# hugocornellier/face_detection_tflite

Measured on NVIDIA B200. Metric: images/sec BlazeFace detect (pre+infer+NMS), higher is better.
Workload: dtype f32

## Files before the change

face_detection_tflite_b200/csrc/engine.cu:

```cuda
#include "engine.h"

#include <algorithm>
#include <cstdio>
#include <cstdlib>

namespace fdt {

Engine::~Engine() {
  if (d_blob_) cudaFree(d_blob_);
  for (TailLayerD* p : d_tail_) if (p) cudaFree(p);
  for (TailBlk* p : d_blks_) if (p) cudaFree(p);
}

bool Engine::init(const uint8_t* tflite, size_t len, int fuse_level, std::string* err, bool use_tc) {
  if (!model_.parse(tflite, len, err)) return false;
  if (!plan_.build(model_, fuse_level, err, use_tc)) return false;
  size_t bytes = plan_.blob.size() * sizeof(float) + 64;
  if (cudaMalloc(&d_blob_, bytes) != cudaSuccess) { *err = "cudaMalloc(weights) failed"; return false; }
  cudaMemset(d_blob_, 0, bytes);
  if (cudaMemcpy(d_blob_, plan_.blob.data(), plan_.blob.size() * sizeof(float), cudaMemcpyHostToDevice) != cudaSuccess) {
    *err = "weight upload failed";
    return false;
  }
  d_tail_.assign(plan_.steps.size(), nullptr);
  d_blks_.assign(plan_.steps.size(), nullptr);
  for (size_t i = 0; i < plan_.steps.size(); ++i) {
    const PStep& st = plan_.steps[i];
    if (st.kind != kStepTailWs) continue;
    if (cudaMalloc(&d_tail_[i], st.tail.size() * sizeof(TailLayerD)) != cudaSuccess ||
        cudaMemcpy(d_tail_[i], st.tail.data(), st.tail.size() * sizeof(TailLayerD), cudaMemcpyHostToDevice) != cudaSuccess) {
      *err = "tail program upload failed";
      return false;
    }
    if (st.tail_blks.empty()) continue;
    if (cudaMalloc(&d_blks_[i], st.tail_blks.size() * sizeof(TailBlk)) != cudaSuccess ||
        cudaMemcpy(d_blks_[i], st.tail_blks.data(), st.tail_blks.size() * sizeof(TailBlk), cudaMemcpyHostToDevice) != cudaSuccess) {
      *err = "chain block table upload failed";
      return false;
    }
  }
  return true;
}

bool Engine::make_ctx(int cap, EngineCtx* ctx, std::string* err) const {
  ctx->cap = cap;
  size_t bytes = (size_t)cap * plan_.arena_per_image * sizeof(float) + 256;
  if (cudaMalloc(&ctx->arena, bytes) != cudaSuccess) { *err = "cudaMalloc(arena) failed"; return false; }
  cudaMemset(ctx->arena, 0, bytes);
  ctx->outputs.clear();
  for (long long e : plan_.out_elems) {
    float* p = nullptr;
    size_t ob = (size_t)cap * e * sizeof(float) + 256;
    if (cudaMalloc(&p, ob) != cudaSuccess) { *err = "cudaMalloc(outputs) failed"; return false; }
    cudaMemset(p, 0, ob);
    ctx->outputs.push_back(p);
  }
  return true;
}

void Engine::free_ctx(EngineCtx* ctx) const {
  if (ctx->arena) cudaFree(ctx->arena);
  for (float* p : ctx->outputs) cudaFree(p);
  ctx->arena = nullptr;
  ctx->outputs.clear();
}

TV Engine::view(const EngineCtx& ctx, int t) const {
  const PTensor& x = plan_.tensors[t];
  TV v;
  v.H = x.H; v.W = x.W; v.C = x.C; v.Cs = x.Cs;
  v.istride = x.istride;
  if (x.root >= 0) v.p = ctx.outputs[x.root] + x.view_off;
  else v.p = ctx.arena + (size_t)x.arena_off * ctx.cap;
  return v;
}

static int cta_cap(size_t smem, int threads) {
  int by_smem = (int)((227u * 1024u) / (smem + 1024u));
  int by_thr = 2048 / std::max(threads, 32);
  int per_sm = std::max(1, std::min(std::min(by_smem, by_thr), 16));
  return 148 * per_sm;
}

int Engine::run(const EngineCtx& ctx, const uint8_t* in_u8, int B, cudaStream_t s, cudaEvent_t* evs) const {
  int launches = 0;
  const float* blob = d_blob_;
  for (const PStep& st : plan_.steps) {
    if (evs) cudaEventRecord(evs[launches], s);
    TV out = view(ctx, st.out);
    switch (st.kind) {
      case kStepNormalize:
        launch_normalize(in_u8, out, B, s);
        break;
      case kStepNaiveConv: {
        NaiveConvP p;
        p.in = view(ctx, st.in); p.out = out;
        p.w = blob + st.w; p.bias = blob + st.bias;
        p.alpha = st.alpha >= 0 ? blob + st.alpha : nullptr;
        p.kh = st.kh; p.kw = st.kw; p.sh = st.sh; p.sw = st.sw; p.pt = st.pt; p.pl = st.pl;
        p.act = st.act; p.depthwise = st.depthwise;
        launch_naive_conv(p, B, s);
        break;
      }
      case kStepStem: {
        StemP p;
        const PTensor& it = plan_.tensors[st.in];
        p.in8 = in_u8; p.H = it.H; p.W = it.W; p.OH = out.H; p.OW = out.W;
        p.kw = st.kw; p.pt = st.pt; p.pl = st.pl; p.K = st.K; p.KP = st.KP;
        p.out = out.p; p.out_istride = out.istride; p.Cout = st.Cout; p.CoutS = out.Cs;
        p.vec_store = (out.Cs % 4 == 0 && out.istride % 4 == 0 && ((size_t)out.p % 16 == 0)) ? ((out.Cs % 8 == 0 && out.istride % 8 == 0 && ((size_t)out.p % 32 == 0)) ? 2 : 1) : 0;
        p.w = blob + st.w; p.bias = blob + st.bias; p.alpha = st.alpha >= 0 ? blob + st.alpha : nullptr;
        p.act = st.act; p.CoutP = st.CoutP; p.NC = st.NC; p.smem_bytes = st.smem;
        launch_stem(p, B, s, cta_cap(st.smem, 32 * (st.NC / 4)));
        break;
      }
      case kStepStemWs: {
        StemWsP p;
        const PTensor& it = plan_.tensors[st.in];
        p.in8 = in_u8; p.H = it.H; p.W = it.W; p.OH = out.H; p.OW = out.W;
        p.kw = st.kw; p.pt = st.pt; p.pl = st.pl;
        p.out = out.p; p.out_istride = out.istride; p.Cout = st.Cout; p.CoutS = out.Cs;
        p.vec_store = (out.Cs % 4 == 0 && out.istride % 4 == 0 && ((size_t)out.p % 16 == 0)) ? ((out.Cs % 8 == 0 && out.istride % 8 == 0 && ((size_t)out.p % 32 == 0)) ? 2 : 1) : 0;
        p.wB = blob + st.w; p.bias = blob + st.bias; p.alpha = st.alpha >= 0 ? blob + st.alpha : nullptr;
        p.act = st.act; p.Npad = st.Npad; p.K8 = st.K8; p.tmem_cols = st.tmem_cols; p.w_parts = st.w_parts;
        p.out_scale = (float)st.out_scale; p.smem_bytes = st.smem;
        if (!launch_stem_ws(p, B, ctx.cap, s)) { failed_ = true; fprintf(stderr, "fdt: cuTensorMapEncodeTiled failed for step '%s'\n", st.name.c_str()); }
        break;
      }
      case kStepGemmConv: {
        GemmConvP p;
        const PTensor& it = plan_.tensors[st.in];
        if (st.in_u8) {
          p.in = nullptr; p.in8 = in_u8; p.in_istride = (long long)it.H * it.W * 4;
          p.Cin = 3; p.CinS = 3;
        } else {
          TV iv = view(ctx, st.in);
          p.in = iv.p; p.in8 = nullptr; p.in_istride = iv.istride; p.Cin = it.C; p.CinS = it.Cs;
        }
        p.H = it.H; p.W = it.W;
        p.kh = st.kh; p.kw = st.kw; p.sh = st.sh; p.sw = st.sw; p.pt = st.pt; p.pl = st.pl;
        p.OH = out.H; p.OW = out.W;
        p.K = st.K; p.KP = st.KP; p.KS = st.KS;
        p.out = out.p; p.out_istride = out.istride; p.Cout = st.Cout; p.CoutS = out.Cs;
        p.vec_store = (out.Cs % 4 == 0 && out.istride % 4 == 0 && ((size_t)out.p % 16 == 0)) ? ((out.Cs % 8 == 0 && out.istride % 8 == 0 && ((size_t)out.p % 32 == 0)) ? 2 : 1) : 0;
        p.w = blob + st.w; p.bias = blob + st.bias; p.alpha = st.alpha >= 0 ? blob + st.alpha : nullptr;
        p.act = st.act; p.CoutP = st.CoutP; p.NC = st.NC; p.nchunks = st.nchunks;
        p.NPG = st.NPG; p.TM = st.TM; p.smem_bytes = st.smem;
        p.flat = (!st.in_u8 && out.H == 1 && out.W == 1 && st.pt == 0 && st.pl == 0 && st.kh == it.H && st.kw == it.W &&
                  it.Cs == it.C && (st.K % 4) == 0 && it.istride % 4 == 0) ? 1 : 0;
        p.fd_KP = FastDiv(st.KP); p.fd_kwc = FastDiv(st.kw * p.Cin); p.fd_Cin = FastDiv(p.Cin);
        p.fd_OW = FastDiv(out.W); p.fd_OH = FastDiv(out.H); p.fd_NQ = FastDiv(st.NC / 4);
        launch_gemm_conv(p, B, s, cta_cap(st.smem, st.NPG * (st.NC / 4)));
        break;
      }
      case kStepDwPw: {
        DwPwP p;
        TV iv = view(ctx, st.in);
        p.in = iv.p; p.in_istride = iv.istride; p.H = iv.H; p.W = iv.W; p.Cin = iv.C; p.CinS = iv.Cs;
        p.has_dw = st.has_dw ? 1 : 0; p.s = st.dws; p.dpt = st.dpt; p.dpl = st.dpl;
        p.OH = out.H; p.OW = out.W;
        p.dww = st.dww >= 0 ? blob + st.dww : nullptr; p.dwb = st.dwb >= 0 ? blob + st.dwb : nullptr;
        p.KP = st.KP; p.KS = st.KS;
        p.out = out.p; p.out_istride = out.istride; p.Cout = st.Cout; p.CoutS = out.Cs;
        p.vec_store = (out.Cs % 4 == 0 && out.istride % 4 == 0 && ((size_t)out.p % 16 == 0)) ? ((out.Cs % 8 == 0 && out.istride % 8 == 0 && ((size_t)out.p % 32 == 0)) ? 2 : 1) : 0;
        p.w = blob + st.w; p.bias = blob + st.bias; p.alpha = st.alpha >= 0 ? blob + st.alpha : nullptr;
        p.act = st.act; p.CoutP = st.CoutP; p.NC = st.NC; p.nchunks = st.nchunks;
        p.NPG = st.NPG; p.TM = st.TM;
        p.res_mode = st.in2 >= 0 ? st.res_mode : 0;
        if (st.in2 >= 0) {
          TV rv = view(ctx, st.in2);
          p.res = rv.p; p.res_istride = rv.istride; p.res_H = rv.H; p.res_W = rv.W; p.res_C = rv.C; p.res_Cs = rv.Cs;
        } else {
          p.res = nullptr; p.res_istride = 0; p.res_H = p.res_W = p.res_C = p.res_Cs = 0;
        }
        p.res_pool = st.res_pool;
        p.TH = st.TH; p.TW = st.TW; p.G = st.G; p.IH = st.IH; p.IW = st.IW; p.tilesX = st.tilesX; p.tilesY = st.tilesY;
        p.fd_Q = FastDiv(st.KP / 4); p.fd_IW = FastDiv(st.IW); p.fd_IH = FastDiv(st.IH); p.fd_TW = FastDiv(st.TW);
        p.fd_thw = FastDiv(st.TH * st.TW); p.fd_NQ = FastDiv(st.NC / 4); p.fd_tpg = FastDiv(st.tilesX * st.tilesY);
        p.fd_tilesX = FastDiv(st.tilesX);
        p.smem_bytes = st.smem;
        launch_dwpw(p, B, s, cta_cap(st.smem, st.NPG * (st.NC / 4)));
        break;
      }
      case kStepBlockWs: {
        DwPwTcP p;
        TV iv = view(ctx, st.in);
        p.in = iv.p; p.in_istride = iv.istride; p.H = iv.H; p.W = iv.W; p.Cin = iv.C; p.CinS = iv.Cs;
        p.has_dw = st.has_dw ? 1 : 0; p.s = st.dws; p.dpt = st.dpt; p.dpl = st.dpl;
        p.OH = out.H; p.OW = out.W;
        p.dww = st.dww >= 0 ? blob + st.dww : nullptr; p.dwb = st.dwb >= 0 ? blob + st.dwb : nullptr;
        p.K8 = st.K8; p.KS = st.KS;
        p.out = out.p; p.out_istride = out.istride; p.Cout = st.Cout; p.CoutS = out.Cs;
        p.vec_store = (out.Cs % 4 == 0 && out.istride % 4 == 0 && ((size_t)out.p % 16 == 0)) ? ((out.Cs % 8 == 0 && out.istride % 8 == 0 && ((size_t)out.p % 32 == 0)) ? 2 : 1) : 0;
        p.wB = blob + st.w; p.bias = blob + st.bias; p.alpha = st.alpha >= 0 ? blob + st.alpha : nullptr;
        p.act = st.act; p.Npad = st.Npad; p.tmem_cols = st.tmem_cols; p.a_rows = st.a_rows; p.RS = st.RS; p.w_parts = st.w_parts; p.nbuf = st.nbuf;
        p.res_mode = st.in2 >= 0 ? st.res_mode : 0;
        if (st.in2 >= 0) {
          TV rv = view(ctx, st.in2);
          p.res = rv.p; p.res_istride = rv.istride; p.res_H = rv.H; p.res_W = rv.W; p.res_C = rv.C; p.res_Cs = rv.Cs;
        } else {
          p.res = nullptr; p.res_istride = 0; p.res_H = p.res_W = p.res_C = p.res_Cs = 0;
        }
        p.res_pool = st.res_pool; p.res_lim = iv.Cs;
        p.TH = st.TH; p.TW = st.TW; p.G = st.G; p.IH = st.IH; p.IW = st.IW; p.tilesX = st.tilesX; p.tilesY = st.tilesY;
        p.fd_Q8 = FastDiv(st.K8 / 4); p.fd_IW = FastDiv(st.IW); p.fd_IH = FastDiv(st.IH); p.fd_TW = FastDiv(st.TW);
        p.fd_thw = FastDiv(st.TH * st.TW); p.fd_tpg = FastDiv(st.tilesX * st.tilesY); p.fd_tilesX = FastDiv(st.tilesX);
        p.fd_nstrips = FastDiv(st.TH / st.RS); p.fd_nslots = FastDiv(st.G * st.TH * st.TW);
        p.n_chunks = st.G * st.IH * st.IW * (st.K8 / 4);
        p.n_items = st.has_dw ? st.G * (st.K8 / 4) * (st.TH / st.RS) * st.TW : 0;
        {
          long long in = (long long)st.G * st.IH * st.IW * st.KS, tail = (long long)(128 - st.a_rows) * st.K8;
          p.in_floats = (int)((std::max(in, tail) + 3) / 4 * 4);
        }
        p.smem_bytes = st.smem;
        p.ns = st.ns; p.na = st.na; p.nd = st.nd; p.nt = st.nt; p.trace = nullptr;
        p.deint = st.deint; p.plane_floats = st.plane_floats; p.PW = st.PW;
        p.nr = st.in2 >= 0 ? st.nr : 0; p.KSr = st.KSr; p.res_stage_floats = st.res_stage_floats;
        p.no = st.no; p.KSo = st.KSo; p.out_stage_floats = st.out_stage_floats;
        p.out2 = nullptr; p.out2_istride = 0; p.Cs2 = 0; p.c1 = 0; p.c2 = 0;
        if (st.out2 >= 0) {
          TV o2 = view(ctx, st.out2);
          p.out2 = o2.p; p.out2_istride = o2.istride; p.Cs2 = o2.Cs; p.c1 = st.c1; p.c2 = st.c2;
          p.Cout = st.c1;
        }
        p.in_floats = st.in_stage_floats;
        if (!launch_block_ws(p, B, ctx.cap, s)) { failed_ = true; fprintf(stderr, "fdt: k_block_ws could not be launched for step '%s'\n", st.name.c_str()); }
        break;
      }
      case kStepTailWs: {
        TailP p;
        TV iv = view(ctx, st.in);
        p.in = iv.p; p.in_istride = iv.istride; p.H = iv.H; p.W = iv.W; p.CinS = iv.Cs;
        p.blob = blob; p.layers = d_tail_[&st - plan_.steps.data()]; p.nlayers = (int)st.tail.size();
        p.nbuf = st.tail_nbuf;
        for (int k = 0; k < kTailMaxBufs; ++k) { p.buf_off[k] = st.tail_buf_off[k]; p.buf_ks[k] = st.tail_buf_ks[k]; }
        p.act_floats = st.tail_act_floats; p.in_bytes = st.tail_in_bytes;
        p.generic = 0;
        for (const TailLayerD& L : st.tail)
          if (L.kind >= 2 || L.act == 2 || L.w_parts != 1 || L.wscale != 1.f || L.rbuf != L.src || (L.kind != 1 && L.o1 >= 0)) p.generic = 1;
        p.blks = nullptr; p.nblks = 0; p.bias_floats = 0; p.in_px = iv.H * iv.W;
        for (int k = 0; k < 2; ++k) { p.rsrc[k] = nullptr; p.rs_istride[k] = 0; p.rs_cs[k] = p.rs_w[k] = p.rs_c[k] = 0; }
        if (st.tail_wide) {
          p.generic = 2;
          p.blks = d_blks_[&st - plan_.steps.data()]; p.nblks = (int)st.tail_blks.size(); p.bias_floats = st.tail_bias_floats;
          for (size_t k = 0; k < st.tail_rsrc.size() && k < 2; ++k) {
            TV rv = view(ctx, st.tail_rsrc[k]);
            p.rsrc[k] = rv.p; p.rs_istride[k] = rv.istride; p.rs_cs[k] = rv.Cs; p.rs_w[k] = rv.W; p.rs_c[k] = rv.C;
          }
        }
        p.last_a_layer = st.tail_last_a; p.wbuf_bytes = st.tail_wbuf; p.wdepth = st.tail_wdepth; p.tbuf_bytes = st.tail_tbuf; p.smem_bytes = st.smem;
        for (int k = 0; k < 4; ++k) { p.outs[k] = nullptr; p.out_istride[k] = 0; p.out_pix[k] = 0; }
        for (size_t k = 0; k < st.tail_outs.size(); ++k) {
          TV ov = view(ctx, st.tail_outs[k]);
          p.outs[k] = ov.p; p.out_istride[k] = ov.istride; p.out_pix[k] = ov.Cs;
        }
        if (!launch_tail_ws(p, B, ctx.cap, s)) { failed_ = true; fprintf(stderr, "fdt: k_tail_ws could not be launched for step '%s'\n", st.name.c_str()); }
        break;
      }
      case kStepFcTc: {
        FcP p;
        TV iv = view(ctx, st.in);
        p.in = iv.p; p.in_istride = iv.istride;
        p.out = out.p; p.out_istride = out.istride;
        p.w = blob + st.w; p.bias = blob + st.bias;
        p.K = st.K; p.K16 = st.K8; p.N = st.Cout; p.w_parts = st.w_parts; p.tile_bytes = st.ts_rec_bytes; p.wscale = (float)st.out_scale;
        if (!launch_fc_tc(p, B, s)) { failed_ = true; fprintf(stderr, "fdt: k_fc_tc could not be launched for step '%s'\n", st.name.c_str()); }
        break;
      }
      case kStepBlockTs: {
        BlockTsP p;
        TV iv = view(ctx, st.in);
        p.in = iv.p; p.in_istride = iv.istride; p.H = iv.H; p.W = iv.W; p.CinS = iv.Cs;
        p.out = out.p; p.out_istride = out.istride; p.OH = out.H; p.OW = out.W; p.CoutS = out.Cs;
        p.rec = blob + st.ts_rec; p.bias = blob + st.ts_bias; p.rec_bytes = st.ts_rec_bytes;
        p.Cin = iv.C; p.K16 = st.ts_k16; p.Npad = st.ts_npad; p.KS = st.ts_ks;
        p.stride = st.dws; p.res = st.ts_res; p.relu = st.ts_relu;
        p.wide = (out.Cs % 8 == 0 && out.istride % 8 == 0 && ((size_t)out.p % 32 == 0)) ? 1 : 0;
        p.ns = st.ts_ns; p.stage_bytes = st.ts_stage_bytes; p.smem_bytes = st.smem;
        {
          const float* hdw = plan_.blob.data() + st.ts_rec + (size_t)st.ts_npad * st.ts_k16 / 2;
          for (int q = 0; q < 16; ++q)
            for (int k = 0; k < 10; ++k)
              for (int c = 0; c < 4; ++c) p.dw[(q * 10 + k) * 4 + c] = 4 * q + c < st.ts_k16 ? hdw[k * st.ts_k16 + 4 * q + c] : 0.f;
        }
        if (!launch_block_ts(p, B, ctx.cap, s)) { failed_ = true; fprintf(stderr, "fdt: k_block_ts could not be launched for step '%s'\n", st.name.c_str()); }
        break;
      }
      case kStepAdd: case kStepAct: case kStepPadC: {
        EltP p;
        p.a = view(ctx, st.in);
        p.b = st.in2 >= 0 ? view(ctx, st.in2) : p.a;
        p.out = out;
        p.alpha = st.alpha >= 0 ? blob + st.alpha : nullptr;
        p.act = st.act;
        if (st.kind == kStepAdd) launch_add(p, B, s);
        else if (st.kind == kStepAct) launch_act(p, B, s);
        else launch_padc(p, B, s);
        break;
      }
      case kStepMaxPool: {
        PoolP p;
        p.in = view(ctx, st.in); p.out = out;
        p.fh = st.fh; p.fw = st.fw; p.sh = st.sh; p.sw = st.sw; p.pt = st.pt; p.pl = st.pl;
        launch_maxpool(p, B, s);
        break;
      }
      case kStepResize: {
        ResizeP p;
        p.in = view(ctx, st.in); p.out = out; p.align_corners = st.align; p.half_pixel = st.half;
        p.has_add = st.in2 >= 0 ? 1 : 0; p.act = st.act;
        p.add = st.in2 >= 0 ? view(ctx, st.in2) : p.in;
        launch_resize_bilinear(p, B, s);
        break;
      }
    }
    ++launches;
  }
  if (evs) cudaEventRecord(evs[launches], s);
  return launches;
}

}
```

face_detection_tflite_b200/csrc/kernels.h:

```cpp
#pragma once
#include <cuda_runtime.h>
#include <algorithm>
#include <cstdint>

#include "../../include/fdt_api.h"
#include "tail_layer.h"

namespace fdt {

enum { kActNone = 0, kActRelu = 1, kActPrelu = 2 };

struct FastDiv {
  unsigned mul = 0, shr = 0, d = 1;
  FastDiv() {}
  explicit FastDiv(int div) {
    d = div < 1 ? 1u : (unsigned)div;
    unsigned l = 0;
    while ((1ull << l) < d) ++l;
    shr = l;
    mul = (unsigned)(((1ull << 32) * ((1ull << l) - d)) / d + 1);
  }
#ifdef __CUDACC__
  __device__ __forceinline__ int div(int n) const { return (int)((__umulhi(mul, (unsigned)n) + (unsigned)n) >> shr); }
  __device__ __forceinline__ void divmod(int n, int& q, int& r) const { q = div(n); r = n - q * (int)d; }
#endif
};

struct TV {
  float* p = nullptr;
  long long istride = 0;
  int H = 1, W = 1, C = 1, Cs = 1;
};

struct NaiveConvP {
  TV in, out;
  const float* w;
  const float* bias;
  const float* alpha;
  int kh, kw, sh, sw, pt, pl, act, depthwise;
};
struct EltP {
  TV a, b, out;
  const float* alpha;
  int act;
};
struct PoolP { TV in, out; int fh, fw, sh, sw, pt, pl; };
struct ResizeP { TV in, out; int align_corners, half_pixel; TV add; int has_add, act; };

void launch_naive_conv(const NaiveConvP& p, int B, cudaStream_t s);
void launch_add(const EltP& p, int B, cudaStream_t s);
void launch_act(const EltP& p, int B, cudaStream_t s);
void launch_padc(const EltP& p, int B, cudaStream_t s);
void launch_maxpool(const PoolP& p, int B, cudaStream_t s);
void launch_resize_bilinear(const ResizeP& p, int B, cudaStream_t s);

#ifdef __CUDACC__
__device__ __forceinline__ int sat_u8(int v) { return v < 0 ? 0 : (v > 255 ? 255 : v); }
__device__ __forceinline__ void yuv_to_bgr(int Y, int U, int V, int* v) {
  const int yy = max(Y - 16, 0) * 1220542 + (1 << 19), u = U - 128, w = V - 128;
  v[0] = sat_u8((yy + 2116026 * u) >> 20);
  v[1] = sat_u8((yy - 852492 * w - 409993 * u) >> 20);
  v[2] = sat_u8((yy + 1673527 * w) >> 20);
}
#endif
struct LetterboxP {
  const uint8_t* frames;
  long long frame_stride;
  int row_stride, channels, src_w, src_h;
  uint8_t* out;
  int dst_w, dst_h, new_w, new_h, pad_top, pad_left;
  const int* x0; const int* x1; const short* ax0; const short* ax1;
  const int* y0; const int* y1; const short* by0; const short* by1;
  int identity;
};
void launch_letterbox(const LetterboxP& p, int B, cudaStream_t s);
struct LetterboxYuvP {
  LetterboxP lb;
  const uint8_t* chroma;
  long long c_frame_stride;
  int c_row_stride, c_step, u_off, v_off;
  const int* cy0; const int* cy1;
};
void launch_letterbox_yuv(const LetterboxYuvP& p, int B, cudaStream_t s);
struct LetterboxTrP {
  LetterboxYuvP yp;
  int yuv;
};
void launch_letterbox_tr(const LetterboxTrP& p, int B, cudaStream_t s);
struct FrameD {
  const uint8_t* y;
  const uint8_t* c;
  int w, h, row_stride;
  int channels;
  int c_row_stride, c_step, u_off, v_off;
  int new_w, new_h, pad_top, pad_left, identity;
  int tx, ty;
  int orientation;
};
struct LetterboxMultiP {
  const FrameD* fr;
  const int* taps;
  uint8_t* out;
  int dst_w, dst_h;
};
void launch_letterbox_multi(const LetterboxMultiP& p, int B, bool transposed, cudaStream_t s);
void launch_normalize(const uint8_t* in, TV out, int B, cudaStream_t s);

struct StemP {
  const uint8_t* in8;
  int H, W, OH, OW, kw, pt, pl, K, KP;
  float* out; long long out_istride; int Cout, CoutS, vec_store;
  const float* w;
  const float* bias; const float* alpha;
  int act, CoutP, NC;
  size_t smem_bytes;
};
void launch_stem(const StemP& p, int B, cudaStream_t s, int max_ctas);

struct GemmConvP {
  const float* in;
  const uint8_t* in8;
  long long in_istride;
  int H, W, Cin, CinS;
  int kh, kw, sh, sw, pt, pl, OH, OW;
  int K, KP, KS;
  float* out; long long out_istride; int Cout, CoutS, vec_store;
  const float* w;
  const float* bias;
  const float* alpha;
  int act, CoutP, NC, nchunks, NPG, TM;
  int flat;
  FastDiv fd_KP, fd_kwc, fd_Cin, fd_OW, fd_OH, fd_NQ;
  size_t smem_bytes;
};
void launch_gemm_conv(const GemmConvP& p, int B, cudaStream_t s, int max_ctas);

struct DwPwP {
  const float* in; long long in_istride; int H, W, Cin, CinS;
  int has_dw, s, dpt, dpl, OH, OW;
  const float* dww;
  const float* dwb;
  int KP, KS;
  float* out; long long out_istride; int Cout, CoutS, vec_store;
  const float* w;
  const float* bias; const float* alpha;
  int act, CoutP, NC, nchunks, NPG, TM;
  const float* res; long long res_istride; int res_H, res_W, res_C, res_Cs, res_pool;
  int res_mode;
  int TH, TW, G, IH, IW, tilesX, tilesY;
  FastDiv fd_Q, fd_IW, fd_IH, fd_TW, fd_thw, fd_NQ, fd_tpg, fd_tilesX;
  size_t smem_bytes;
};
void launch_dwpw(const DwPwP& p, int B, cudaStream_t s, int max_ctas);

struct DwPwTcP {
  const float* in; long long in_istride; int H, W, Cin, CinS;
  int has_dw, s, dpt, dpl, OH, OW;
  const float* dww;
  const float* dwb;
  int K8, KS;
  float* out; long long out_istride; int Cout, CoutS, vec_store;
  const float* wB;
  const float* bias; const float* alpha;
  int act, Npad, tmem_cols, a_rows, RS;
  int in_floats, n_chunks, n_items;
  int nr, KSr, res_stage_floats;
  int deint, plane_floats, PW;
  int w_parts;
  int nbuf;
  int ns, na, nd, nt;
  int no, KSo, out_stage_floats;
  float* out2; long long out2_istride; int Cs2, c1, c2;
  long long* trace;
  const float* res; long long res_istride; int res_H, res_W, res_C, res_Cs, res_pool, res_mode, res_lim;
  int TH, TW, G, IH, IW, tilesX, tilesY;
  FastDiv fd_Q8, fd_IW, fd_IH, fd_TW, fd_thw, fd_tpg, fd_tilesX, fd_nstrips, fd_nslots;
  size_t smem_bytes;
};
bool launch_block_ws(const DwPwTcP& p, int B, int cap, cudaStream_t s);

struct StemWsP {
  const uint8_t* in8;
  int H, W, OH, OW, kw, pt, pl;
  float* out; long long out_istride; int Cout, CoutS, vec_store;
  const float* wB;
  const float* bias; const float* alpha;
  int act, Npad, K8, tmem_cols, w_parts;
  float out_scale;
  size_t smem_bytes;
};
bool launch_stem_ws(const StemWsP& p, int B, int cap, cudaStream_t s);

struct BlockTsP {
  const float* in; long long in_istride; int H, W, CinS;
  float* out; long long out_istride; int OH, OW, CoutS;
  const float* rec;
  const float* bias;
  int rec_bytes;
  int Cin, K16, Npad, KS;
  int stride;
  int res;
  int relu, wide;
  int ns, stage_bytes;
  size_t smem_bytes;
  alignas(16) float dw[10 * 64];
};
size_t ts_smem_bytes(int rec_bytes, int Npad, int ns, int stage_bytes);
bool launch_block_ts(const BlockTsP& p, int B, int cap, cudaStream_t s);

struct TailP {
  const float* in; long long in_istride; int H, W, CinS;
  const float* blob;
  const TailLayerD* layers;
  int nlayers;
  int nbuf;
  int buf_off[kTailMaxBufs];
  int buf_ks[kTailMaxBufs];
  int act_floats;
  int in_bytes;
  int last_a_layer;
  int wbuf_bytes, wdepth;
  int tbuf_bytes;
  int generic;
  const TailBlk* blks; int nblks; int bias_floats; int in_px;
  const float* rsrc[2]; long long rs_istride[2]; int rs_cs[2], rs_w[2], rs_c[2];
  float* outs[4]; long long out_istride[4]; int out_pix[4];
  size_t smem_bytes;
};
size_t tail_smem_bytes(int act_floats, int wbuf_bytes, int wdepth, int tbuf_bytes);
size_t wide_smem_bytes(int act_floats, int wbuf_bytes, int wdepth, int tbuf_bytes, int bias_floats);
bool launch_tail_ws(const TailP& p, int B, int cap, cudaStream_t s);

struct FcP {
  const float* in; long long in_istride;
  float* out; long long out_istride;
  const float* w;
  const float* bias;
  int K, K16, N, w_parts, tile_bytes;
  float wscale;
};
bool launch_fc_tc(const FcP& p, int B, cudaStream_t s);

struct JpegIdctP {
  const int16_t* coef;
  const uint16_t* q;
  int bw, bh;
  uint8_t* plane; int pitch;
};
struct JpegColorP {
  const uint8_t* py; const uint8_t* pcb; const uint8_t* pcr;
  int pitch_y, pitch_c;
  int W, H, ncomp;
  int cdw, cdh, hs, vs;
  int orientation;
  uint8_t* out; int out_w;
};
void launch_jpeg_idct(const JpegIdctP& p, cudaStream_t s);
void launch_jpeg_color(const JpegColorP& p, cudaStream_t s);

struct DecodeP {
  const float* boxes; long long boxes_istride;
  const float* scores; long long scores_istride;
  const double* anchors;
  int N, input_h;
  double raw_thresh, score_thresh, iou_thresh;
  double pad_t, pad_b, pad_l, pad_r;
  double min_score, min_face_size, img_w, img_h;
  int max_faces;
  fdt_face* faces;
  int* counts;
  int* cand_idx; int cand_cap; int* cand_n;
  const double* pre;
  double* dbg_dec;
  int skip_roi;
  const double* geom = nullptr;
};
size_t decode_smem_bytes(int N);
void launch_decode_nms(const DecodeP& p, int B, cudaStream_t s);

struct WarpP {
  const uint8_t* frames; long long frame_stride; int row_stride, channels, src_w, src_h;
  const int* crop_img;
  const double* affine;
  int ncrops, out_size;
  int flip_odd;
  uint8_t* crops;
  int yuv = 0;
  long long c_off = 0;
  int c_row_stride = 0, c_step = 0, u_off = 0, v_off = 0;
  const FrameD* fr = nullptr;
  int orientation = 1;
};
void launch_warp_affine(const WarpP& p, cudaStream_t s);

struct MeshPostP {
  const float* raw; long long raw_istride;
  const float* flag; long long flag_istride;
  const double* roi;
  int nfaces, in_size;
  float* mesh_out;
  double* score_out;
  double* eye_corners;
};
void launch_mesh_post(const MeshPostP& p, cudaStream_t s);

struct IrisPostP {
  const float* contours; long long contours_istride;
  const float* iris; long long iris_istride;
  const double* roi;
  int nfaces, in_size;
  double img_w, img_h;
  const double* img_wh = nullptr;
  float* iris_out;
  double* eye_kp;
};
void launch_iris_post(const IrisPostP& p, cudaStream_t s);

}
```

face_detection_tflite_b200/csrc/kernels_tail.cu:

```cuda
#include <cuda.h>
#include <cuda_fp16.h>

#include <algorithm>
#include <cstdio>
#include <map>
#include <mutex>
#include <tuple>

#include "kernels.h"

namespace fdt {
namespace {

#ifndef FDT_TAIL_WARPS
#define FDT_TAIL_WARPS 12
#endif
constexpr int kTC = FDT_TAIL_WARPS;
constexpr int kTG = kTC / 4;
constexpr int kTComputeThreads = kTC * 32;
constexpr int kTThreads = (kTC + 1) * 32;
__device__ __forceinline__ uint32_t col_d(int t) { return t ? 128u : 0u; }
__device__ __forceinline__ uint32_t col_a(int t) { return t ? 384u : 256u; }
constexpr uint32_t kLBO = 128;

__device__ __forceinline__ uint32_t smem_u32(const void* p) { return (uint32_t)__cvta_generic_to_shared(p); }
__device__ __forceinline__ void mbar_init(uint32_t bar, uint32_t count) { asm volatile("mbarrier.init.shared::cta.b64 [%0], %1;" ::"r"(bar), "r"(count)); }
__device__ __forceinline__ void mbar_arrive(uint32_t bar) { asm volatile("mbarrier.arrive.shared::cta.b64 _, [%0];" ::"r"(bar) : "memory"); }
__device__ __forceinline__ void mbar_expect_tx(uint32_t bar, uint32_t bytes) {
  asm volatile("mbarrier.arrive.expect_tx.shared::cta.b64 _, [%0], %1;" ::"r"(bar), "r"(bytes) : "memory");
}
__device__ __forceinline__ void mbar_wait(uint32_t bar, uint32_t parity) {
  uint32_t ok = 0;
  while (!ok)
    asm volatile("{\n\t.reg .pred p;\n\tmbarrier.try_wait.parity.shared::cta.b64 p, [%1], %2;\n\tselp.u32 %0, 1, 0, p;\n\t}\n"
                 : "=r"(ok) : "r"(bar), "r"(parity) : "memory");
}
__device__ __forceinline__ void mbar_wait_idle(uint32_t bar, uint32_t parity) {
  uint32_t ok = 0;
  while (!ok)
    asm volatile("{\n\t.reg .pred p;\n\tmbarrier.try_wait.parity.shared::cta.b64 p, [%1], %2, %3;\n\tselp.u32 %0, 1, 0, p;\n\t}\n"
                 : "=r"(ok) : "r"(bar), "r"(parity), "r"(0x989680u) : "memory");
}
__device__ __forceinline__ float4 lds4(uint32_t addr) {
  float4 v;
  asm("ld.shared.v4.f32 {%0, %1, %2, %3}, [%4];" : "=f"(v.x), "=f"(v.y), "=f"(v.z), "=f"(v.w) : "r"(addr) : "memory");
  return v;
}
__device__ __forceinline__ void sts4(uint32_t addr, const float4& v) {
  asm volatile("st.shared.v4.f32 [%0], {%1, %2, %3, %4};" ::"r"(addr), "f"(v.x), "f"(v.y), "f"(v.z), "f"(v.w) : "memory");
}
__device__ __forceinline__ void fma4(float4& a, const float4& v, const float4& w) {
  asm("{\n\t.reg .b64 ra, rv, rw;\n\t"
      "mov.b64 ra, {%0, %1};\n\tmov.b64 rv, {%4, %5};\n\tmov.b64 rw, {%8, %9};\n\t"
      "fma.rn.f32x2 ra, rv, rw, ra;\n\tmov.b64 {%0, %1}, ra;\n\t"
      "mov.b64 ra, {%2, %3};\n\tmov.b64 rv, {%6, %7};\n\tmov.b64 rw, {%10, %11};\n\t"
      "fma.rn.f32x2 ra, rv, rw, ra;\n\tmov.b64 {%2, %3}, ra;\n\t}"
      : "+f"(a.x), "+f"(a.y), "+f"(a.z), "+f"(a.w)
      : "f"(v.x), "f"(v.y), "f"(v.z), "f"(v.w), "f"(w.x), "f"(w.y), "f"(w.z), "f"(w.w));
}
__device__ __forceinline__ float4 max4(const float4& a, const float4& b) {
  return make_float4(fmaxf(a.x, b.x), fmaxf(a.y, b.y), fmaxf(a.z, b.z), fmaxf(a.w, b.w));
}
__device__ __forceinline__ uint32_t pack_h2(float e0, float e1) {
  uint32_t d;
  asm("cvt.rn.satfinite.f16x2.f32 %0, %1, %2;" : "=r"(d) : "f"(e1), "f"(e0));
  return d;
}
__device__ __forceinline__ void split_store_tmem(uint32_t taddr_hi, const float4& a) {
  const uint32_t h0 = pack_h2(a.x, a.y), h1 = pack_h2(a.z, a.w);
  const __half2 hh0 = *reinterpret_cast<const __half2*>(&h0), hh1 = *reinterpret_cast<const __half2*>(&h1);
  const float2 f0 = __half22float2(hh0), f1 = __half22float2(hh1);
  const uint32_t l0 = pack_h2(a.x - f0.x, a.y - f0.y), l1 = pack_h2(a.z - f1.x, a.w - f1.y);
  asm volatile("tcgen05.st.sync.aligned.32x32b.x2.b32 [%0], {%1, %2};" ::"r"(taddr_hi), "r"(h0), "r"(h1) : "memory");
  asm volatile("tcgen05.st.sync.aligned.32x32b.x2.b32 [%0], {%1, %2};" ::"r"(taddr_hi + 64u), "r"(l0), "r"(l1) : "memory");
}
__device__ __forceinline__ void mma_ts_f16(uint32_t tmem_d, uint32_t tmem_a, uint32_t b_lo, uint32_t b_hi, uint32_t idesc, uint32_t acc) {
  asm volatile(
      "{\n\t.reg .pred p;\n\t.reg .b64 db;\n\tmov.b64 db, {%2, %3};\n\tsetp.ne.b32 p, %5, 0;\n\t"
      "tcgen05.mma.cta_group::1.kind::f16 [%0], [%1], db, %4, p;\n\t}\n" ::"r"(tmem_d), "r"(tmem_a), "r"(b_lo), "r"(b_hi), "r"(idesc), "r"(acc));
}

#ifdef FDT_TAIL_TRACE
#define TT(k) do { if (blockIdx.x == 0 && tid == 0 && it == 1) tt[l * 6 + (k)] = clock64(); } while (0)
#else
#define TT(k) do { } while (0)
#endif
template <bool GEN>
__global__ void __launch_bounds__(kTThreads, 1) k_tail_ws(const __grid_constant__ CUtensorMap tmap, const __grid_constant__ TailP p, int B) {
#ifdef FDT_TAIL_TRACE
  __shared__ long long tt[16 * 6];
#endif
  extern __shared__ __align__(128) unsigned char smem_raw[];
  __shared__ uint32_t tmem_base_s;
  const int tid = threadIdx.x, warp = tid >> 5, lane = tid & 31;
  TailLayerD* sL = reinterpret_cast<TailLayerD*>(smem_raw);
  float* sBias = reinterpret_cast<float*>(smem_raw + kTailMaxLayers * sizeof(TailLayerD));
  float* sAlpha = sBias + kTailMaxLayers * 128;
  uint64_t* bars = reinterpret_cast<uint64_t*>(sAlpha + kTailMaxLayers * 128);
  float* scratch = reinterpret_cast<float*>(bars + 16);
  float* act0 = reinterpret_cast<float*>((reinterpret_cast<uintptr_t>(scratch + 16) + 127) & ~(uintptr_t)127);
  float* zslot = act0 + p.act_floats;
  unsigned char* tring = reinterpret_cast<unsigned char*>((reinterpret_cast<uintptr_t>(zslot + 128) + 127) & ~(uintptr_t)127);
  unsigned char* wring = tring + 2 * (size_t)p.tbuf_bytes;
  const uint32_t bar0 = smem_u32(bars);
  const uint32_t in_full = bar0, a_free = bar0 + 8u, w_full = bar0 + 16u, a_full = bar0 + 32u, d_full = bar0 + 48u, t_full = bar0 + 56u;
  const int nl = p.nlayers;
  const int my_images = blockIdx.x < B ? (B - 1 - (int)blockIdx.x) / (int)gridDim.x + 1 : 0;

  for (int i = tid; i < nl * (int)(sizeof(TailLayerD) / 16); i += kTThreads)
    reinterpret_cast<uint4*>(sL)[i] = reinterpret_cast<const uint4*>(p.layers)[i];
  for (int i = (p.in_bytes >> 2) + tid; i < p.act_floats + 128; i += kTThreads) act0[i] = 0.f;
  if (warp == kTC) {
    if (lane == 0) {
      mbar_init(in_full, 1);
      mbar_init(a_free, kTC);
      for (int i = 0; i < 2; ++i) { mbar_init(w_full + 8u * i, 1); mbar_init(a_full + 8u * i, kTC); mbar_init(t_full + 8u * i, 1); }
      mbar_init(d_full, 1);
      asm volatile("fence.mbarrier_init.release.cluster;" ::: "memory");
      asm volatile("prefetch.tensormap [%0];" ::"l"(&tmap) : "memory");
    }
    __syncwarp();
    asm volatile("tcgen05.alloc.cta_group::1.sync.aligned.shared::cta.b32 [%0], %1;" ::"r"(smem_u32(&tmem_base_s)), "r"(512u));
    asm volatile("tcgen05.relinquish_alloc_permit.cta_group::1.sync.aligned;" ::);
  }
  __syncthreads();
  for (int l = 0; l < nl; ++l)
    for (int i = tid; i < sL[l].Npad; i += kTThreads) {
      sBias[l * 128 + i] = p.blob[(size_t)sL[l].bias_off + i];
      if (GEN && sL[l].act == 2) sAlpha[l * 128 + i] = p.blob[(size_t)sL[l].alpha_off + i];
    }
  asm volatile("tcgen05.fence::before_thread_sync;" ::: "memory");
  __syncthreads();
  asm volatile("tcgen05.fence::after_thread_sync;" ::: "memory");
  const uint32_t tmem_base = tmem_base_s;
  const uint32_t act_a = smem_u32(act0), zero_a = smem_u32(zslot), wring_a = smem_u32(wring), tring_a = smem_u32(tring);

  if (warp < kTC) {
    const int lq = warp & 3, g = warp >> 2;
    const int r = lq * 32 + lane;
    const uint32_t tm_lane = tmem_base + ((uint32_t)(lq * 32) << 16);
    uint32_t ph_d = 0u, ph_t0 = 0u, ph_t1 = 0u;
    int gl = 0, it = 0;
    for (int img = blockIdx.x; img < B; img += gridDim.x, ++it) {
      mbar_wait(in_full, (uint32_t)(it & 1));
      for (int l = 0; l < nl; ++l, ++gl) {
        const TailLayerD L = sL[l];
        TT(0);
        const uint32_t src_a = act_a + 4u * (uint32_t)p.buf_off[L.src], kss_b = 4u * (uint32_t)p.buf_ks[L.src];
        const uint32_t dst_a = L.dst >= 0 ? act_a + 4u * (uint32_t)p.buf_off[L.dst] : 0u, ksd_b = L.dst >= 0 ? 4u * (uint32_t)p.buf_ks[L.dst] : 0u;
        const int src_q = (int)(kss_b >> 4), dst_q = (int)(ksd_b >> 4);
        const int npix = L.OH * L.OW;
        const uint32_t tb_a = tring_a + (uint32_t)(gl & 1) * (uint32_t)p.tbuf_bytes;
        if (L.tap_bytes) {
          if (gl & 1) { mbar_wait(t_full + 8u, ph_t1); ph_t1 ^= 1u; } else { mbar_wait(t_full, ph_t0); ph_t0 ^= 1u; }
        }
        TT(1);
        if (GEN && L.kind == 3) {
          const int n = npix * L.Cin;
          float sacc = 0.f;
          for (int i = tid; i < n; i += kTComputeThreads) {
            const int px = i / L.Cin, c = i - px * L.Cin;
            float a, w;
            asm("ld.shared.f32 %0, [%1];" : "=f"(a) : "r"(src_a + (uint32_t)px * kss_b + 4u * (uint32_t)c) : "memory");
            asm("ld.shared.f32 %0, [%1];" : "=f"(w) : "r"(tb_a + 4u * (uint32_t)i) : "memory");
            sacc = fmaf(a, w, sacc);
          }
#pragma unroll
          for (int o = 16; o > 0; o >>= 1) sacc += __shfl_xor_sync(0xffffffffu, sacc, o);
          if (lane == 0) { scratch[warp] = sacc; mbar_arrive(a_full); mbar_arrive(a_full + 8u); }
          asm volatile("bar.sync 1, %0;" ::"n"(kTComputeThreads) : "memory");
          if (tid == 0) {
            float tot = sBias[l * 128];
            for (int w2 = 0; w2 < kTC; ++w2) tot += scratch[w2];
            p.outs[L.o1][(size_t)img * p.out_istride[L.o1]] = tot;
          }
          asm volatile("bar.sync 1, %0;" ::"n"(kTComputeThreads) : "memory");
          if (l == p.last_a_layer && lane == 0) mbar_arrive(a_free);
          continue;
        }
        const bool paired = npix > 128;
        const int ntiles = paired ? 2 : 1;
        const int rows = paired ? (npix >> 1) : npix;
        const int nq = L.K16 >> 2, nq_real = (L.Cin + 3) >> 2, nq_half = (L.K16 >> 5) << 2;
        const uint32_t dww_a = tb_a, dwb_a = dww_a + 9u * (uint32_t)L.K16 * 4u;
        const uint32_t k16_b = (uint32_t)L.K16 * 4u;
        const uint32_t acol0 = tm_lane + col_a(0), acol1 = tm_lane + col_a(1);
        int oy = r / L.OW;
        const int ox = r - oy * L.OW;
        if (paired) oy *= 2;
        const bool act = r < rows;
        const bool warp_on = lq * 32 < rows;
        const int pix0 = oy * L.OW + ox;
        bool half_done = false;
        if (!warp_on) {
        } else if (L.kind == 0) {
          uint32_t off[12];
          const int iy0 = oy * L.stride - L.pad, ix0 = ox * L.stride - L.pad;
#pragma unroll
          for (int k = 0; k < 12; ++k) {
            const int iy = iy0 + k / 3, ix = ix0 + k % 3;
            const bool ok = act && (unsigned)iy < (unsigned)L.IH && (unsigned)ix < (unsigned)L.IW;
            off[k] = ok ? src_a + (uint32_t)(iy * L.IW + ix) * kss_b : zero_a;
          }
          for (int q = g; q < nq; q += kTG) {
            if (!half_done && q >= nq_half) {
              half_done = true;
              asm volatile("tcgen05.wait::st.sync.aligned;" ::: "memory");
              asm volatile("tcgen05.fence::before_thread_sync;" ::: "memory");
              __syncwarp();
              if (lane == 0) mbar_arrive(a_full);
            }
            float4 a0 = make_float4(0.f, 0.f, 0.f, 0.f), a1 = a0;
            if (q < nq_real) {
              const uint32_t qo = 16u * (uint32_t)q;
              float4 w[9];
#pragma unroll
              for (int k = 0; k < 9; ++k) w[k] = lds4(dww_a + (uint32_t)k * k16_b + qo);
              const float4 bias = lds4(dwb_a + qo);
              float4 v[3];
#pragma unroll
              for (int c = 0; c < 3; ++c) v[c] = lds4(off[c] + qo);
              a0 = bias;
#pragma unroll
              for (int c = 0; c < 3; ++c) fma4(a0, v[c], w[c]);
#pragma unroll
              for (int c = 0; c < 3; ++c) v[c] = lds4(off[3 + c] + qo);
              a1 = bias;
#pragma unroll
              for (int c = 0; c < 3; ++c) { fma4(a0, v[c], w[3 + c]); if (paired) fma4(a1, v[c], w[c]); }
#pragma unroll
              for (int c = 0; c < 3; ++c) v[c] = lds4(off[6 + c] + qo);
#pragma unroll
              for (int c = 0; c < 3; ++c) { fma4(a0, v[c], w[6 + c]); if (paired) fma4(a1, v[c], w[3 + c]); }
              if (paired) {
#pragma unroll
                for (int c = 0; c < 3; ++c) v[c] = lds4(off[9 + c] + qo);
#pragma unroll
                for (int c = 0; c < 3; ++c) fma4(a1, v[c], w[6 + c]);
              }
            }
            split_store_tmem(acol0 + 2u * (uint32_t)q, a0);
            if (paired) split_store_tmem(acol1 + 2u * (uint32_t)q, a1);
          }
        } else {
          const uint32_t px0 = act ? src_a + (uint32_t)pix0 * kss_b : zero_a;
          const uint32_t px1 = px0 + (uint32_t)L.OW * kss_b;
          for (int q = g; q < nq; q += kTG) {
            if (!half_done && q >= nq_half) {
              half_done = true;
              asm volatile("tcgen05.wait::st.sync.aligned;" ::: "memory");
              asm volatile("tcgen05.fence::before_thread_sync;" ::: "memory");
              __syncwarp();
              if (lane == 0) mbar_arrive(a_full);
            }
            const bool in = q < src_q;
            split_store_tmem(acol0 + 2u * (uint32_t)q, in ? lds4(px0 + 16u * (uint32_t)q) : make_float4(0.f, 0.f, 0.f, 0.f));
            if (paired) split_store_tmem(acol1 + 2u * (uint32_t)q, in ? lds4(px1 + 16u * (uint32_t)q) : make_float4(0.f, 0.f, 0.f, 0.f));
          }
        }
        if (warp_on) asm volatile("tcgen05.wait::st.sync.aligned;" ::: "memory");
        TT(2);
        asm volatile("tcgen05.fence::before_thread_sync;" ::: "memory");
        __syncwarp();
        if (lane == 0) { if (!half_done) mbar_arrive(a_full); mbar_arrive(a_full + 8u); }
        if (warp_on) {
          const uint32_t bias_a = smem_u32(sBias + l * 128), alpha_a = smem_u32(sAlpha + l * 128);
          const uint32_t rsrc_a = GEN ? act_a + 4u * (uint32_t)p.buf_off[L.rbuf] : src_a, ksr_b = GEN ? 4u * (uint32_t)p.buf_ks[L.rbuf] : kss_b;
          const int res_q = (int)(ksr_b >> 4);
          mbar_wait(d_full, ph_d);
          TT(3);
          asm volatile("tcgen05.fence::after_thread_sync;" ::: "memory");
          const uint32_t row_b = (uint32_t)L.IW * ksr_b;
#pragma unroll 1
          for (int t = 0; t < ntiles; ++t) {
            const int pix = pix0 + t * L.OW;
            const uint32_t dcol = tm_lane + col_d(t);
            uint32_t res_a = zero_a;
            if (act && L.res == 1) res_a = rsrc_a + (uint32_t)pix * ksr_b;
            if (act && L.res == 2) res_a = rsrc_a + (uint32_t)((2 * oy) * L.IW + 2 * ox) * ksr_b;
            const uint32_t out_a = dst_a + (uint32_t)(act ? pix : 0) * ksd_b;
            float* o1 = nullptr; float* o2 = nullptr;
            int o1_q = 0;
            if (GEN ? L.o1 >= 0 : L.kind == 1) {
              o1 = p.outs[L.o1] + (size_t)img * p.out_istride[L.o1] + (size_t)(act ? pix : 0) * p.out_pix[L.o1];
              o1_q = p.out_pix[L.o1] >> 2;
              if (L.o2 >= 0) o2 = p.outs[L.o2] + (size_t)img * p.out_istride[L.o2] + (size_t)(act ? pix : 0) * p.out_pix[L.o2];
            }
            for (int c16 = g; c16 < (L.Npad >> 4); c16 += kTG) {
              uint32_t u[16];
              asm volatile(
                  "tcgen05.ld.sync.aligned.32x32b.x16.b32 {%0, %1, %2, %3, %4, %5, %6, %7, %8, %9, %10, %11, %12, %13, %14, %15}, [%16];"
                  : "=r"(u[0]), "=r"(u[1]), "=r"(u[2]), "=r"(u[3]), "=r"(u[4]), "=r"(u[5]), "=r"(u[6]), "=r"(u[7]),
                    "=r"(u[8]), "=r"(u[9]), "=r"(u[10]), "=r"(u[11]), "=r"(u[12]), "=r"(u[13]), "=r"(u[14]), "=r"(u[15])
                  : "r"(dcol + 16u * (uint32_t)c16));
              float4 bv[4], rv[4];
#pragma unroll
              for (int j = 0; j < 4; ++j) {
                const int cq = 4 * c16 + j;
                const uint32_t qo = 16u * (uint32_t)cq;
                bv[j] = lds4(bias_a + qo);
                rv[j] = make_float4(0.f, 0.f, 0.f, 0.f);
                if (L.res == 1) {
                  if (cq < res_q) rv[j] = lds4(res_a + qo);
                } else if (L.res == 2) {
                  if (cq < res_q) rv[j] = max4(max4(lds4(res_a + qo), lds4(res_a + ksr_b + qo)), max4(lds4(res_a + row_b + qo), lds4(res_a + row_b + ksr_b + qo)));
                }
              }
              asm volatile("tcgen05.wait::ld.sync.aligned;" ::: "memory");
#pragma unroll
              for (int j = 0; j < 4; ++j) {
                const int cq = 4 * c16 + j;
                float4 v;
                if (GEN) v = make_float4(fmaf(__uint_as_float(u[4 * j]), L.wscale, bv[j].x), fmaf(__uint_as_float(u[4 * j + 1]), L.wscale, bv[j].y),
                                         fmaf(__uint_as_float(u[4 * j + 2]), L.wscale, bv[j].z), fmaf(__uint_as_float(u[4 * j + 3]), L.wscale, bv[j].w));
                else v = make_float4(__uint_as_float(u[4 * j]) + bv[j].x, __uint_as_float(u[4 * j + 1]) + bv[j].y,
                                     __uint_as_float(u[4 * j + 2]) + bv[j].z, __uint_as_float(u[4 * j + 3]) + bv[j].w);
                if (L.kind != 1) {
                  v.x += rv[j].x; v.y += rv[j].y; v.z += rv[j].z; v.w += rv[j].w;
                  if (L.act == 1) {
                    v = max4(v, make_float4(0.f, 0.f, 0.f, 0.f));
                  } else if (GEN && L.act == 2) {
                    const float4 al = lds4(alpha_a + 16u * (uint32_t)cq);
                    v = make_float4(fmaf(al.x, fminf(v.x, 0.f), fmaxf(v.x, 0.f)), fmaf(al.y, fminf(v.y, 0.f), fmaxf(v.y, 0.f)),
                                    fmaf(al.z, fminf(v.z, 0.f), fmaxf(v.z, 0.f)), fmaf(al.w, fminf(v.w, 0.f), fmaxf(v.w, 0.f)));
                  }
                  if (act && cq < dst_q) sts4(out_a + 16u * (uint32_t)cq, v);
                  if (GEN && act && cq < o1_q) *reinterpret_cast<float4*>(o1 + 4 * cq) = v;
                } else if (act) {
                  const int c = 4 * cq;
                  if (c + 4 <= L.c1) {
                    *reinterpret_cast<float4*>(o1 + c) = v;
                  } else {
                    const float vv[4] = {v.x, v.y, v.z, v.w};
#pragma unroll
                    for (int e = 0; e < 4; ++e)
                      if (c + e >= L.c1 && c + e - L.c1 < L.c2) o2[c + e - L.c1] = vv[e];
                  }
                }
              }
            }
          }
        }
        ph_d ^= 1u;
        TT(4);
        asm volatile("tcgen05.fence::before_thread_sync;" ::: "memory");
        asm volatile("bar.sync 1, %0;" ::"n"(kTComputeThreads) : "memory");
        TT(5);
        asm volatile("tcgen05.fence::after_thread_sync;" ::: "memory");
        if (l == p.last_a_layer && lane == 0) mbar_arrive(a_free);
      }
#ifdef FDT_TAIL_TRACE
      if (blockIdx.x == 0 && tid == 0 && it == 1)
        for (int l2 = 0; l2 < nl; ++l2)
          printf("tail layer %2d: taps-wait %5lld  depthwise %6lld  mma-wait %5lld  epilogue %5lld  barrier %5lld  | total %6lld\n", l2, tt[l2 * 6 + 1] - tt[l2 * 6],
                 tt[l2 * 6 + 2] - tt[l2 * 6 + 1], tt[l2 * 6 + 3] - tt[l2 * 6 + 2], tt[l2 * 6 + 4] - tt[l2 * 6 + 3], tt[l2 * 6 + 5] - tt[l2 * 6 + 4],
                 tt[l2 * 6 + 5] - tt[l2 * 6]);
#endif
    }
  } else if (lane == 0) {
    const int total = my_images * nl;
    const int D = p.wdepth;
    auto load_weights = [&](int glayer) {
      const TailLayerD& L = sL[glayer % nl];
      if (!L.rec_bytes) return;
      const uint32_t slot = (uint32_t)(glayer % D), bar = w_full + 8u * slot;
      mbar_expect_tx(bar, (uint32_t)L.rec_bytes);
      asm volatile("cp.async.bulk.shared::cluster.global.mbarrier::complete_tx::bytes [%0], [%1], %2, [%3];"
                   ::"r"(wring_a + slot * (uint32_t)p.wbuf_bytes), "l"(p.blob + (size_t)L.rec_off), "r"((uint32_t)L.rec_bytes), "r"(bar) : "memory");
    };
    auto load_taps = [&](int glayer) {
      const TailLayerD& L = sL[glayer % nl];
      if (!L.tap_bytes) return;
      const uint32_t slot = (uint32_t)(glayer & 1), bar = t_full + 8u * slot;
      mbar_expect_tx(bar, (uint32_t)L.tap_bytes);
      asm volatile("cp.async.bulk.shared::cluster.global.mbarrier::complete_tx::bytes [%0], [%1], %2, [%3];"
// ... 570 lines not shown
```

face_detection_tflite_b200/csrc/kernels_ts.cu:

```cuda
#include <cuda.h>
#include <cuda_fp16.h>

#include <algorithm>
#include <cstdio>
#include <map>
#include <mutex>
#include <tuple>
#include <type_traits>

#include "kernels.h"
#include "tile_walk.h"

namespace fdt {
namespace {

constexpr int kC = 12;
constexpr int kThreads = (kC + 2) * 32;
constexpr uint32_t kLBO = 128;

__device__ __forceinline__ uint32_t smem_u32(const void* p) { return (uint32_t)__cvta_generic_to_shared(p); }
__device__ __forceinline__ void mbar_init(uint32_t bar, uint32_t count) { asm volatile("mbarrier.init.shared::cta.b64 [%0], %1;" ::"r"(bar), "r"(count)); }
__device__ __forceinline__ void mbar_arrive(uint32_t bar) { asm volatile("mbarrier.arrive.shared::cta.b64 _, [%0];" ::"r"(bar) : "memory"); }
__device__ __forceinline__ void mbar_expect_tx(uint32_t bar, uint32_t bytes) {
  asm volatile("mbarrier.arrive.expect_tx.shared::cta.b64 _, [%0], %1;" ::"r"(bar), "r"(bytes) : "memory");
}
__device__ __forceinline__ void mbar_wait(uint32_t bar, uint32_t parity) {
  uint32_t ok = 0;
  while (!ok)
    asm volatile("{\n\t.reg .pred p;\n\tmbarrier.try_wait.parity.shared::cta.b64 p, [%1], %2;\n\tselp.u32 %0, 1, 0, p;\n\t}\n"
                 : "=r"(ok) : "r"(bar), "r"(parity) : "memory");
}
__device__ __forceinline__ void mbar_wait_idle(uint32_t bar, uint32_t parity) {
  uint32_t ok = 0;
  while (!ok)
    asm volatile("{\n\t.reg .pred p;\n\tmbarrier.try_wait.parity.shared::cta.b64 p, [%1], %2, %3;\n\tselp.u32 %0, 1, 0, p;\n\t}\n"
                 : "=r"(ok) : "r"(bar), "r"(parity), "r"(0x989680u) : "memory");
}
__device__ __forceinline__ float4 lds4(uint32_t addr) {
  float4 v;
  asm volatile("ld.shared.v4.f32 {%0, %1, %2, %3}, [%4];" : "=f"(v.x), "=f"(v.y), "=f"(v.z), "=f"(v.w) : "r"(addr));
  return v;
}
__device__ __forceinline__ void fma4(float4& a, const float4& v, const float4& w) {
  asm("{\n\t.reg .b64 ra, rv, rw;\n\t"
      "mov.b64 ra, {%0, %1};\n\tmov.b64 rv, {%4, %5};\n\tmov.b64 rw, {%8, %9};\n\t"
      "fma.rn.f32x2 ra, rv, rw, ra;\n\tmov.b64 {%0, %1}, ra;\n\t"
      "mov.b64 ra, {%2, %3};\n\tmov.b64 rv, {%6, %7};\n\tmov.b64 rw, {%10, %11};\n\t"
      "fma.rn.f32x2 ra, rv, rw, ra;\n\tmov.b64 {%2, %3}, ra;\n\t}"
      : "+f"(a.x), "+f"(a.y), "+f"(a.z), "+f"(a.w)
      : "f"(v.x), "f"(v.y), "f"(v.z), "f"(v.w), "f"(w.x), "f"(w.y), "f"(w.z), "f"(w.w));
}
__device__ __forceinline__ float4 max4(const float4& a, const float4& b) {
  return make_float4(fmaxf(a.x, b.x), fmaxf(a.y, b.y), fmaxf(a.z, b.z), fmaxf(a.w, b.w));
}
__device__ __forceinline__ uint32_t pack_h2(float e0, float e1) {
  uint32_t d;
  asm("cvt.rn.satfinite.f16x2.f32 %0, %1, %2;" : "=r"(d) : "f"(e1), "f"(e0));
  return d;
}
__device__ __forceinline__ void split_store_tmem(uint32_t taddr_hi, uint32_t lo_off, const float4& a) {
  const uint32_t h0 = pack_h2(a.x, a.y), h1 = pack_h2(a.z, a.w);
  const float2 f0 = __half22float2(*reinterpret_cast<const __half2*>(&h0)), f1 = __half22float2(*reinterpret_cast<const __half2*>(&h1));
  const uint32_t l0 = pack_h2(a.x - f0.x, a.y - f0.y), l1 = pack_h2(a.z - f1.x, a.w - f1.y);
  asm volatile("tcgen05.st.sync.aligned.32x32b.x2.b32 [%0], {%1, %2};" ::"r"(taddr_hi), "r"(h0), "r"(h1) : "memory");
  asm volatile("tcgen05.st.sync.aligned.32x32b.x2.b32 [%0], {%1, %2};" ::"r"(taddr_hi + lo_off), "r"(l0), "r"(l1) : "memory");
}
__device__ __forceinline__ void mma_ts_f16(uint32_t tmem_d, uint32_t tmem_a, uint32_t b_lo, uint32_t b_hi, uint32_t idesc, uint32_t acc) {
  asm volatile(
      "{\n\t.reg .pred p;\n\t.reg .b64 db;\n\tmov.b64 db, {%2, %3};\n\tsetp.ne.b32 p, %5, 0;\n\t"
      "tcgen05.mma.cta_group::1.kind::f16 [%0], [%1], db, %4, p;\n\t}\n" ::"r"(tmem_d), "r"(tmem_a), "r"(b_lo), "r"(b_hi), "r"(idesc), "r"(acc));
}
__device__ __forceinline__ void stg8(float* p, const float4& a, const float4& b) {
  asm volatile("st.global.v8.f32 [%0], {%1, %2, %3, %4, %5, %6, %7, %8};" ::"l"(p), "f"(a.x), "f"(a.y), "f"(a.z), "f"(a.w), "f"(b.x), "f"(b.y), "f"(b.z), "f"(b.w) : "memory");
}

__device__ __forceinline__ uint32_t col_d(int slot, int t) { return (uint32_t)(slot * 2 + t) * 64u; }
__device__ __forceinline__ uint32_t col_a(int slot, int t) { return 256u + (uint32_t)(slot * 2 + t) * 64u; }

template <int S, int KSC>
__global__ void __launch_bounds__(kThreads, 1) k_block_ts(const __grid_constant__ CUtensorMap tmap, const __grid_constant__ BlockTsP p, int B) {
  extern __shared__ __align__(128) unsigned char smem_raw[];
  __shared__ uint32_t tmem_base_s;
  constexpr int NT = S == 1 ? 2 : 1;
  constexpr int TH = S == 1 ? 16 : 8, TW = 16;
  constexpr int IW = S == 1 ? 18 : 17;
  const int tid = threadIdx.x, warp = tid >> 5, lane = tid & 31;
  float* sRec = reinterpret_cast<float*>(smem_raw);
  float* sBias = sRec + (p.rec_bytes >> 2);
  uint64_t* bars = reinterpret_cast<uint64_t*>(sBias + p.Npad);
  unsigned char* ring = reinterpret_cast<unsigned char*>((reinterpret_cast<uintptr_t>(bars + 32) + 127) & ~(uintptr_t)127);
  const uint32_t bar0 = smem_u32(bars);
  const uint32_t in_full = bar0, in_empty = bar0 + 64u, a_full = bar0 + 128u, d_full = bar0 + 144u;
  const int NS = p.ns;
  const int tiles_x = p.OW / TW, tiles_y = p.OH / TH, tpi = tiles_x * tiles_y;
  const int ntiles = B * tpi;
  const int n_my = (int)blockIdx.x < ntiles ? (ntiles - 1 - (int)blockIdx.x) / (int)gridDim.x + 1 : 0;

  for (int i = tid; i < (p.rec_bytes >> 4); i += kThreads) reinterpret_cast<uint4*>(sRec)[i] = reinterpret_cast<const uint4*>(p.rec)[i];
  for (int i = tid; i < p.Npad; i += kThreads) sBias[i] = p.bias[i];
  if (tid < 2) bars[24 + tid] = 0ull;
  if (tid == 0) {
    for (int i = 0; i < NS; ++i) { mbar_init(in_full + 8u * i, 1); mbar_init(in_empty + 8u * i, kC); }
    for (int i = 0; i < 2; ++i) { mbar_init(a_full + 8u * i, kC); mbar_init(d_full + 8u * i, 1); }
    asm volatile("fence.mbarrier_init.release.cluster;" ::: "memory");
    asm volatile("prefetch.tensormap [%0];" ::"l"(&tmap) : "memory");
  }
  if (warp == kC + 1) {
    asm volatile("tcgen05.alloc.cta_group::1.sync.aligned.shared::cta.b32 [%0], %1;" ::"r"(smem_u32(&tmem_base_s)), "r"(512u));
    asm volatile("tcgen05.relinquish_alloc_permit.cta_group::1.sync.aligned;" ::);
  }
  asm volatile("fence.proxy.async.shared::cta;" ::: "memory");
  asm volatile("tcgen05.fence::before_thread_sync;" ::: "memory");
  __syncthreads();
  asm volatile("tcgen05.fence::after_thread_sync;" ::: "memory");
  const uint32_t tmem_base = tmem_base_s;
  const int KS = KSC ? KSC : p.KS;
  const uint32_t ring_a = smem_u32(ring), ks_b = (uint32_t)KS * 4u, row_b = (uint32_t)IW * ks_b;
  const uint32_t stage_b = (uint32_t)p.stage_bytes;
  const uint32_t plane_b = (17u * 17u * ks_b + 127u) & ~127u;
  const uint32_t col2_b[3] = {0u, plane_b, ks_b};

  if (warp < kC) {
    const int lq = warp & 3, g = warp >> 2;
    const int L = lq * 32 + lane;
    const int yy = L >> 4, x = L & 15;
    const uint32_t tm_lane = tmem_base + ((uint32_t)(lq * 32) << 16);
    const uint32_t win = (uint32_t)((2 * yy) * IW + x) * ks_b;
    const int nq = p.K16 >> 2, nq_real = (p.Cin + 3) >> 2, ks_q = KS >> 2;
    const uint32_t bias_a = smem_u32(sBias), zero_a = bar0 + 192u;
    const int couts = p.CoutS, nc8 = (couts + 7) >> 3;
    const int gw = (nc8 + 2) / 3, g0 = gw * g, gn = max(0, min(gw, nc8 - g0));

    float4 rvp[3][2];
    auto epilogue = [&](int i, int stage, int b, int ty, int tx) {
      const int slot = i & 1;
      mbar_wait(d_full + 8u * (uint32_t)slot, (uint32_t)((i >> 1) & 1));
      asm volatile("tcgen05.fence::after_thread_sync;" ::: "memory");
      const uint32_t st_a = ring_a + (uint32_t)stage * stage_b + win;
      float* const orow0 = p.out + (size_t)b * p.out_istride + (uint32_t)(((ty * TH + (S == 1 ? 2 * yy : yy)) * p.OW + tx * TW + x) * couts);
      const uint32_t orow_step = (uint32_t)(p.OW * couts);
#pragma unroll
      for (int t = 0; t < NT; ++t) {
        float* orow = orow0 + (t ? orow_step : 0u);
        const uint32_t res_a = S == 1 ? st_a + (uint32_t)(t + 1) * row_b + ks_b : st_a;
        const uint32_t dcol = tm_lane + col_d(slot, t);
        auto unit = [&](auto ngc, auto lgc, int c8) {
          constexpr int NG = decltype(ngc)::value;
          constexpr int lg = decltype(lgc)::value;
          uint32_t u[8 * NG];
          if (NG == 2)
            asm volatile(
                "tcgen05.ld.sync.aligned.32x32b.x16.b32 {%0, %1, %2, %3, %4, %5, %6, %7, %8, %9, %10, %11, %12, %13, %14, %15}, [%16];"
                : "=r"(u[0]), "=r"(u[1]), "=r"(u[2]), "=r"(u[3]), "=r"(u[4]), "=r"(u[5]), "=r"(u[6]), "=r"(u[7]),
                  "=r"(u[8 * (NG - 1)]), "=r"(u[8 * (NG - 1) + 1]), "=r"(u[8 * (NG - 1) + 2]), "=r"(u[8 * (NG - 1) + 3]),
                  "=r"(u[8 * (NG - 1) + 4]), "=r"(u[8 * (NG - 1) + 5]), "=r"(u[8 * (NG - 1) + 6]), "=r"(u[8 * (NG - 1) + 7])
                : "r"(dcol + 8u * (uint32_t)c8));
          else
            asm volatile("tcgen05.ld.sync.aligned.32x32b.x8.b32 {%0, %1, %2, %3, %4, %5, %6, %7}, [%8];"
                         : "=r"(u[0]), "=r"(u[1]), "=r"(u[2]), "=r"(u[3]), "=r"(u[4]), "=r"(u[5]), "=r"(u[6]), "=r"(u[7])
                         : "r"(dcol + 8u * (uint32_t)c8));
          float4 bv[2 * NG], rv[2 * NG];
#pragma unroll
          for (int j = 0; j < 2 * NG; ++j) {
            const int cq = 2 * c8 + j;
            const uint32_t qo = 16u * (uint32_t)cq;
            bv[j] = lds4(bias_a + qo);
            rv[j] = make_float4(0.f, 0.f, 0.f, 0.f);
            if (S == 2) {
              rv[j] = rvp[lg + (j >> 1)][j & 1];
            } else if (S == 1) {
              rv[j] = lds4(p.res == 1 && cq < ks_q ? res_a + qo : zero_a);
            } else if (p.res == 2) {
              if (cq < ks_q) rv[j] = max4(max4(lds4(res_a + qo), lds4(res_a + plane_b + qo)), max4(lds4(res_a + row_b + qo), lds4(res_a + row_b + plane_b + qo)));
            }
          }
          asm volatile("tcgen05.wait::ld.sync.aligned;" ::: "memory");
          float4 v[2 * NG];
#pragma unroll
          for (int j = 0; j < 2 * NG; ++j) {
            v[j] = make_float4(__uint_as_float(u[4 * j]) + bv[j].x + rv[j].x, __uint_as_float(u[4 * j + 1]) + bv[j].y + rv[j].y,
                               __uint_as_float(u[4 * j + 2]) + bv[j].z + rv[j].z, __uint_as_float(u[4 * j + 3]) + bv[j].w + rv[j].w);
            if (p.relu) v[j] = max4(v[j], make_float4(0.f, 0.f, 0.f, 0.f));
          }
#pragma unroll
          for (int k = 0; k < NG; ++k) {
            const int c = 8 * (c8 + k);
            if (c + 8 <= couts) {
              if (p.wide) stg8(orow + c, v[2 * k], v[2 * k + 1]);
              else { *reinterpret_cast<float4*>(orow + c) = v[2 * k]; *reinterpret_cast<float4*>(orow + c + 4) = v[2 * k + 1]; }
            } else if (c + 4 <= couts) {
              *reinterpret_cast<float4*>(orow + c) = v[2 * k];
            }
          }
        };
        if (gn >= 2) unit(std::integral_constant<int, 2>(), std::integral_constant<int, 0>(), g0);
        if (gn == 1) unit(std::integral_constant<int, 1>(), std::integral_constant<int, 0>(), g0);
        if (gn == 3) unit(std::integral_constant<int, 1>(), std::integral_constant<int, 2>(), g0 + 2);
      }
      asm volatile("tcgen05.fence::before_thread_sync;" ::: "memory");
      __syncwarp();
      if (S == 1 && lane == 0) mbar_arrive(in_empty + 8u * (uint32_t)stage);
    };

    const TileStep step = tile_step((int)gridDim.x, tpi, tiles_x);
    TileAt at = tile_at((int)blockIdx.x, tpi, tiles_x), at_prev = at;
    int stage = 0, stage_prev = 0;
    uint32_t in_phase = 0;
    for (int i = 0; i < n_my; ++i) {
      const int slot = i & 1;
      mbar_wait(in_full + 8u * (uint32_t)stage, in_phase);
      const uint32_t st_a = ring_a + (uint32_t)stage * stage_b + win;
      const uint32_t acol0 = tm_lane + col_a(slot, 0), acol1 = tm_lane + col_a(slot, 1);
      for (int q = g; q < nq; q += 3) {
        if (q >= nq_real && i >= 2) break;
        float4 a0 = make_float4(0.f, 0.f, 0.f, 0.f), a1 = a0;
        if (q < nq_real) {
          const uint32_t qo = 16u * (uint32_t)q;
          const float4* cw = reinterpret_cast<const float4*>(p.dw) + 10 * q;
          float4 w[9];
#pragma unroll
          for (int k = 0; k < 9; ++k) w[k] = cw[k];
          const float4 bias = cw[9];
          const uint32_t pa = st_a + qo;
          if (S == 1) {
            float4 v[3];
#pragma unroll
            for (int c = 0; c < 3; ++c) v[c] = lds4(pa + (uint32_t)c * ks_b);
            a0 = bias;
#pragma unroll
            for (int c = 0; c < 3; ++c) fma4(a0, v[c], w[c]);
#pragma unroll
            for (int c = 0; c < 3; ++c) v[c] = lds4(pa + row_b + (uint32_t)c * ks_b);
            a1 = bias;
#pragma unroll
            for (int c = 0; c < 3; ++c) { fma4(a0, v[c], w[3 + c]); fma4(a1, v[c], w[c]); }
#pragma unroll
            for (int c = 0; c < 3; ++c) v[c] = lds4(pa + 2u * row_b + (uint32_t)c * ks_b);
#pragma unroll
            for (int c = 0; c < 3; ++c) { fma4(a0, v[c], w[6 + c]); fma4(a1, v[c], w[3 + c]); }
#pragma unroll
            for (int c = 0; c < 3; ++c) v[c] = lds4(pa + 3u * row_b + (uint32_t)c * ks_b);
#pragma unroll
            for (int c = 0; c < 3; ++c) fma4(a1, v[c], w[6 + c]);
          } else {
            a0 = bias;
#pragma unroll
            for (int k = 0; k < 9; ++k) fma4(a0, lds4(pa + (uint32_t)(k / 3) * row_b + col2_b[k % 3]), w[k]);
          }
        }
        split_store_tmem(acol0 + 2u * (uint32_t)q, 32u, a0);
        if (S == 1) split_store_tmem(acol1 + 2u * (uint32_t)q, 32u, a1);
      }
      asm volatile("tcgen05.wait::st.sync.aligned;" ::: "memory");
      asm volatile("tcgen05.fence::before_thread_sync;" ::: "memory");
      __syncwarp();
      if (lane == 0) mbar_arrive(a_full + 8u * (uint32_t)slot);
      if (i > 0) epilogue(i - 1, stage_prev, at_prev.b, at_prev.ty, at_prev.tx);
      if (S == 2) {
#pragma unroll
        for (int c8i = 0; c8i < 3; ++c8i)
#pragma unroll
          for (int j = 0; j < 2; ++j) {
            const int cq = 2 * (g0 + c8i) + j;
            const uint32_t qo = 16u * (uint32_t)cq;
            rvp[c8i][j] = make_float4(0.f, 0.f, 0.f, 0.f);
            if (p.res == 2 && c8i < gn && cq < ks_q)
              rvp[c8i][j] = max4(max4(lds4(st_a + qo), lds4(st_a + plane_b + qo)), max4(lds4(st_a + row_b + qo), lds4(st_a + row_b + plane_b + qo)));
          }
        __syncwarp();
        if (lane == 0) mbar_arrive(in_empty + 8u * (uint32_t)stage);
      }
      at_prev = at; stage_prev = stage;
      tile_advance(at, step, tiles_x, tiles_y);
      if (++stage == NS) { stage = 0; in_phase ^= 1u; }
    }
    if (n_my > 0) epilogue(n_my - 1, stage_prev, at_prev.b, at_prev.ty, at_prev.tx);
  } else if (warp == kC) {
    if (lane == 0) {
      const TileStep step = tile_step((int)gridDim.x, tpi, tiles_x);
      TileAt at = tile_at((int)blockIdx.x, tpi, tiles_x);
      int stage = 0;
      uint32_t empty_phase = 1;
      for (int i = 0; i < n_my; ++i) {
        const int b = at.b, ty = at.ty, tx = at.tx;
        if (i >= NS) mbar_wait_idle(in_empty + 8u * (uint32_t)stage, empty_phase);
        const uint32_t bar = in_full + 8u * (uint32_t)stage;
        mbar_expect_tx(bar, (uint32_t)((S == 1 ? 18 * 18 : 2 * 17 * 17) * KS) * 4u);
        const int ix0 = S == 1 ? tx * TW - 1 : tx * TW * 2, iy0 = S == 1 ? ty * TH - 1 : ty * TH * 2;
        asm volatile("cp.async.bulk.tensor.4d.shared::cluster.global.mbarrier::complete_tx::bytes [%0], [%1, {%2, %3, %4, %5}], [%6];"
                     ::"r"(ring_a + (uint32_t)stage * stage_b), "l"(&tmap), "r"(0), "r"(ix0), "r"(iy0), "r"(b), "r"(bar) : "memory");
        if (S == 2)
          asm volatile("cp.async.bulk.tensor.4d.shared::cluster.global.mbarrier::complete_tx::bytes [%0], [%1, {%2, %3, %4, %5}], [%6];"
                       ::"r"(ring_a + (uint32_t)stage * stage_b + plane_b), "l"(&tmap), "r"(0), "r"(ix0 + 1), "r"(iy0), "r"(b), "r"(bar) : "memory");
        tile_advance(at, step, tiles_x, tiles_y);
        if (++stage == NS) { stage = 0; empty_phase ^= 1u; }
      }
    }
    __syncwarp();
  } else {
    if (lane == 0) {
      const uint32_t idesc = (1u << 4) | ((uint32_t)(p.Npad >> 3) << 17) | ((128u >> 4) << 24);
      const uint32_t sbo = (uint32_t)(p.K16 >> 3) * 128u;
      const uint32_t b_hi = ((sbo >> 4) & 0x3FFFu) | (1u << 14);
      const uint32_t b_lo0 = ((smem_u32(sRec) & 0x3FFFFu) >> 4) | ((kLBO >> 4) << 16);
      const int ksteps = p.K16 >> 4;
      for (int i = 0; i < n_my; ++i) {
        const int slot = i & 1;
        mbar_wait_idle(a_full + 8u * (uint32_t)slot, (uint32_t)((i >> 1) & 1));
        asm volatile("tcgen05.fence::after_thread_sync;" ::: "memory");
#pragma unroll
        for (int t = 0; t < NT; ++t) {
          const uint32_t dcol = tmem_base + col_d(slot, t), acol = tmem_base + col_a(slot, t);
          uint32_t acc = 0u;
#pragma unroll 1
          for (int part = 0; part < 2; ++part)
#pragma unroll 1
            for (int ks = 0; ks < ksteps; ++ks) {
              mma_ts_f16(dcol, acol + 32u * (uint32_t)part + 8u * (uint32_t)ks, b_lo0 + 16u * (uint32_t)ks, b_hi, idesc, acc);
              acc = 1u;
            }
        }
        asm volatile("tcgen05.commit.cta_group::1.mbarrier::arrive::one.shared::cluster.b64 [%0];" ::"r"(d_full + 8u * (uint32_t)slot) : "memory");
      }
    }
    __syncwarp();
  }
  asm volatile("tcgen05.fence::before_thread_sync;" ::: "memory");
  __syncthreads();
  if (warp == kC + 1) {
    asm volatile("tcgen05.fence::after_thread_sync;" ::: "memory");
    asm volatile("tcgen05.dealloc.cta_group::1.sync.aligned.b32 %0, %1;" ::"r"(tmem_base), "r"(512u));
  }
}

typedef CUresult (*EncodeTiledFn)(CUtensorMap*, CUtensorMapDataType, cuuint32_t, void*, const cuuint64_t*, const cuuint64_t*,
                                  const cuuint32_t*, const cuuint32_t*, CUtensorMapInterleave, CUtensorMapSwizzle,
                                  CUtensorMapL2promotion, CUtensorMapFloatOOBfill);

EncodeTiledFn encode_fn() {
  static EncodeTiledFn fn = [] {
    void* f = nullptr;
    cudaDriverEntryPointQueryResult q;
    if (cudaGetDriverEntryPoint("cuTensorMapEncodeTiled", &f, cudaEnableDefault, &q) != cudaSuccess || q != cudaDriverEntryPointSuccess) f = nullptr;
    return (EncodeTiledFn)f;
  }();
  return fn;
}

bool ts_tensor_map(const BlockTsP& p, int cap, CUtensorMap* out) {
  typedef std::tuple<const void*, int, int, int, int, int, int, long long> Key;
  static std::mutex mu;
  static std::map<Key, CUtensorMap> cache;
  Key key(p.in, cap, p.H, p.W, p.CinS, p.KS, p.stride, p.in_istride);
  std::lock_guard<std::mutex> g(mu);
  auto it = cache.find(key);
  if (it != cache.end()) { *out = it->second; return true; }
  EncodeTiledFn enc = encode_fn();
  if (!enc) return false;
  cuuint64_t gdim[4] = {(cuuint64_t)p.CinS, (cuuint64_t)p.W, (cuuint64_t)p.H, (cuuint64_t)cap};
  cuuint64_t gstr[3] = {(cuuint64_t)p.CinS * 4, (cuuint64_t)p.W * p.CinS * 4, (cuuint64_t)p.in_istride * 4};
  cuuint32_t box[4] = {(cuuint32_t)p.KS, p.stride == 1 ? 18u : 33u, p.stride == 1 ? 18u : 17u, 1u};
  cuuint32_t estr[4] = {1, p.stride == 1 ? 1u : 2u, 1, 1};
  CUtensorMap tm;
  CUresult r = enc(&tm, CU_TENSOR_MAP_DATA_TYPE_FLOAT32, 4, const_cast<float*>(p.in), gdim, gstr, box, estr,
                   CU_TENSOR_MAP_INTERLEAVE_NONE, CU_TENSOR_MAP_SWIZZLE_NONE, CU_TENSOR_MAP_L2_PROMOTION_L2_128B,
                   CU_TENSOR_MAP_FLOAT_OOB_FILL_NONE);
  if (r != CUDA_SUCCESS) return false;
  if (cache.size() > 256) cache.clear();
  cache[key] = tm;
  *out = tm;
  return true;
}

template <int S, int KSC>
bool launch_ts(const CUtensorMap& tm, const BlockTsP& p, int B, cudaStream_t s) {
  static std::mutex mu;
  static std::map<int, size_t> cur;
  int dev = 0, sms = 148;
  cudaGetDevice(&dev);
  cudaDeviceGetAttribute(&sms, cudaDevAttrMultiProcessorCount, dev);
  {
    std::lock_guard<std::mutex> g(mu);
    size_t& c = cur[dev];
    if (p.smem_bytes > c) {
      if (cudaFuncSetAttribute(k_block_ts<S, KSC>, cudaFuncAttributeMaxDynamicSharedMemorySize, (int)p.smem_bytes) != cudaSuccess) return false;
      c = p.smem_bytes;
    }
  }
  const int ntiles = B * (p.OW / 16) * (p.OH / (S == 1 ? 16 : 8));
  const int grid = std::max(1, std::min(ntiles, sms));
  k_block_ts<S, KSC><<<grid, kThreads, p.smem_bytes, s>>>(tm, p, B);
  return true;
}

}

size_t ts_smem_bytes(int rec_bytes, int Npad, int ns, int stage_bytes) {
  return (size_t)rec_bytes + (size_t)Npad * 4 + 32 * 8 + 128 + (size_t)ns * stage_bytes + 128;
}

bool launch_block_ts(const BlockTsP& p, int B, int cap, cudaStream_t s) {
  if (B <= 0) return true;
  CUtensorMap tm;
  if (!ts_tensor_map(p, cap, &tm)) return false;
  if (p.stride == 1) {
    switch (p.KS) {
      case 28: return launch_ts<1, 28>(tm, p, B, s);
      case 36: return launch_ts<1, 36>(tm, p, B, s);
      case 44: return launch_ts<1, 44>(tm, p, B, s);
      case 52: return launch_ts<1, 52>(tm, p, B, s);
      default: return launch_ts<1, 0>(tm, p, B, s);
    }
  }
  switch (p.KS) {
    case 28: return launch_ts<2, 28>(tm, p, B, s);
    case 36: return launch_ts<2, 36>(tm, p, B, s);
    case 44: return launch_ts<2, 44>(tm, p, B, s);
    case 52: return launch_ts<2, 52>(tm, p, B, s);
    default: return launch_ts<2, 0>(tm, p, B, s);
  }
}

}
```

face_detection_tflite_b200/csrc/plan.cpp:

```cpp
#include "plan.h"

#include <algorithm>
#include <cmath>
#include <cstdio>
#include <cstdlib>
#include <cstring>
#include <cstdint>

namespace fdt {
namespace {

constexpr size_t kSmemLimit = 200 * 1024;
constexpr int kActNone = 0, kActRelu = 1, kActPrelu = 2;

inline int ru(int v, int m) { return (v + m - 1) / m * m; }
inline int smem_stride(int KP) { return KP + (((KP / 4) % 2 == 0) ? 4 : 0); }

void same_pad(int in, int k, int s, int* before) {
  int out = (in + s - 1) / s;
  int total = (out - 1) * s + k - in;
  if (total < 0) total = 0;
  *before = total / 2;
}

// ... 122 lines not shown
    if (padded > v.size()) P.blob.insert(P.blob.end(), padded - v.size(), 0.f);
    return off;
  }

  int sole_consumer(int t) const {
    if (ncons[t] != 1) return -1;
    auto c = m.consumers(t);
    return c.size() == 1 ? c[0] : -1;
  }

  void fuse_activation(int* cur, int* act, int* alpha_tf, std::vector<int>* absorbed) {
    if (is_view(*cur)) return;
    int c = sole_consumer(*cur);
    if (c < 0 || done[c]) return;
    const TfOp& op = m.ops[c];
    if (op.code == kOpRelu) {
      *act = kActRelu;
    } else if (op.code == kOpPrelu) {
      std::vector<float> a;
      if (!m.const_f32(op.in[1], &a) || (int)a.size() != m.tensors[*cur].shape.back()) return;
      *act = kActPrelu;
      *alpha_tf = op.in[1];
    } else {
      return;
    }
    absorbed->push_back(c);
    *cur = op.out[0];
  }

  bool pack_alpha(int alpha_tf, size_t padded, long long* off) {
    std::vector<float> a;
    if (!m.const_f32(alpha_tf, &a)) return fail("PRELU alpha is not constant");
    *off = push(a, padded);
    return true;
  }

  static void plan_columns(PStep* s) {
    s->CoutP = ru(s->Cout, 4);
    int quads = s->CoutP / 4;
    s->nchunks = (quads + 23) / 24;
    int nq = (quads + s->nchunks - 1) / s->nchunks;
    s->NC = nq * 4;
    s->TM = nq <= 12 ? 4 : 8;
    s->NPG = 128 / s->TM;
  }

  struct PwMatch {
    bool has_dw = false;
    int dws = 1, dpt = 0, dpl = 0;
    int src = -1, cur = -1, res = -1, pool = 0, act = kActNone, alpha_tf = -1;
    std::vector<int> absorbed;
  };
  bool match_pointwise(int ci, PwMatch* M, bool graph_only) {
    const TfOp& conv = m.ops[ci];
    if (conv.code != kOpConv2D || conv.in.size() < 2) return false;
    const TfTensor& wt = m.tensors[conv.in[1]];
    if (wt.shape.size() != 4 || wt.shape[1] != 1 || wt.shape[2] != 1) return false;
    if (conv.stride_h != 1 || conv.stride_w != 1 || (conv.act != 0 && conv.act != 1)) return false;
    int X = conv.in[0];
    M->src = X;
    int dwi = m.producer(X);
    if (dwi >= 0 && !done[dwi] && m.ops[dwi].code == kOpDwConv2D && ncons[X] == 1 && !is_view(X)) {
      const TfOp& dw = m.ops[dwi];
      const TfTensor& dwt = m.tensors[dw.in[1]];
      bool ok = dwt.shape.size() == 4 && dwt.shape[1] == 3 && dwt.shape[2] == 3 && dw.depth_mult == 1 &&
                dw.dil_h == 1 && dw.dil_w == 1 && dw.padding == 0 && dw.stride_h == dw.stride_w &&
                (dw.stride_h == 1 || dw.stride_h == 2) && dw.act == 0 && dw.in.size() >= 3;
      if (ok) {
        M->has_dw = true;
        M->dws = dw.stride_h;
        M->src = dw.in[0];
        const TfTensor& it = m.tensors[M->src];
        same_pad(it.dim(1), 3, M->dws, &M->dpt);
        same_pad(it.dim(2), 3, M->dws, &M->dpl);
        M->absorbed.push_back(dwi);
      }
    }
    const int Cout = wt.shape[0];
    int cur = conv.out[0];
    M->act = conv.act == 1 ? kActRelu : kActNone;
    if (M->act == kActNone && !is_view(cur)) {
      int c = sole_consumer(cur);
      if (c >= 0 && !done[c] && m.ops[c].code == kOpAdd && (m.ops[c].act == 0 || m.ops[c].act == 1) &&
          m.ops[c].in.size() == 2) {
        const TfOp& add = m.ops[c];
        int R = add.in[0] == cur ? add.in[1] : add.in[0];
        std::vector<int> abs2;
        int r = R;
        int pool = 0;
        bool good = R != cur;
        int pp = m.producer(r);
        if (good && pp >= 0 && m.ops[pp].code == kOpPad && ncons[r] == 1 && !is_view(r) && !done[pp]) {
          std::vector<int> pads;
          const TfTensor& pi = m.tensors[m.ops[pp].in[0]];
          if (m.const_i32(m.ops[pp].in[1], &pads) && pads.size() == 8 && pads[0] == 0 && pads[1] == 0 &&
              pads[2] == 0 && pads[3] == 0 && pads[4] == 0 && pads[5] == 0 && pads[6] == 0 && pi.shape.size() == 4) {
            abs2.push_back(pp);
            r = m.ops[pp].in[0];
            pp = m.producer(r);
          }
        }
        if (good && pp >= 0 && m.ops[pp].code == kOpMaxPool && ncons[r] == 1 && !is_view(r) && !done[pp]) {
          const TfOp& mp = m.ops[pp];
          if (mp.filter_h == 2 && mp.filter_w == 2 && mp.stride_h == 2 && mp.stride_w == 2 && mp.act == 0) {
            abs2.push_back(pp);
            r = mp.in[0];
            pool = 1;
          }
        }
        const TfTensor& rt = m.tensors[r];
        const TfTensor& ot = m.tensors[cur];
        int rp = m.producer(r);
        bool produced_before = graph_only || (rp >= 0 && rp < ci && (!done[rp] || is_output_of_fused(r)));
        good = good && rt.shape.size() == 4 && rt.dim(3) <= Cout && produced_before;
        if (good) {
          if (pool) good = (rt.dim(1) + 1) / 2 == ot.dim(1) && (rt.dim(2) + 1) / 2 == ot.dim(2);
          else good = rt.dim(1) == ot.dim(1) && rt.dim(2) == ot.dim(2);
        }
        if (good) {
          M->res = r;
          M->pool = pool;
          M->absorbed.push_back(c);
          for (int a : abs2) M->absorbed.push_back(a);
          cur = add.out[0];
          if (add.act == 1) M->act = kActRelu;
        }
      }
      if (M->act == kActNone) fuse_activation(&cur, &M->act, &M->alpha_tf, &M->absorbed);
    }
    M->cur = cur;
    return true;
  }

  bool analyse_pointwise(int ci, Fused* F) {
    const TfOp& conv = m.ops[ci];
    PwMatch M;
    if (!match_pointwise(ci, &M, false)) return false;
    const TfTensor& wt = m.tensors[conv.in[1]];
    PStep st;
    st.kind = kStepDwPw;
    std::vector<int> absorbed = M.absorbed;
    const int src = M.src;
    st.has_dw = M.has_dw; st.dws = M.dws; st.dpt = M.dpt; st.dpl = M.dpl;
    const TfTensor& st_in = m.tensors[src];
    if (st_in.shape.size() != 4) return false;
    if (is_view(src) && (st_in.dim(3) % 4 != 0 || views[src].off % 4 != 0 || P.out_elems[views[src].root] % 4 != 0))
      return false;
    int Cin = st_in.dim(3);
    st.Cout = wt.shape[0];
    st.K = Cin;
    st.KP = ru(Cin, 4);
    st.KS = smem_stride(st.KP);
    plan_columns(&st);
    int cur = M.cur;
    int res = M.res, alpha_tf = M.alpha_tf;
    st.act = M.act;
    if (res >= 0) {
      const TfTensor& rt = m.tensors[res];
      st.res_pool = M.pool;
      bool even = rt.dim(1) % 2 == 0 && rt.dim(2) % 2 == 0;
      st.res_mode = (st.has_dw && res == src && (!M.pool || (even && st.dws == 2))) ? 1 : 2;
    }
    const TfTensor& ot = m.tensors[conv.out[0]];
    int OH = ot.dim(1), OW = ot.dim(2);
    if (!plan_spatial(&st, OH, OW)) return false;
    for (int a : absorbed) done[a] = 1;
    done[ci] = 1;
    F->ok = true;
    F->st = st;
    F->src_tf = src;
    F->res_tf = res;
    F->out_tf = cur;
    F->st.name = m.tensors[cur].name;
    fused_outputs.push_back(cur);
    std::vector<float> w, b;
    if (!m.const_f32(conv.in[1], &w)) return fail("conv weights are not constant");
    if (conv.in.size() > 2 && conv.in[2] >= 0) { if (!m.const_f32(conv.in[2], &b)) return fail("conv bias is not constant"); }
    b.resize(st.Cout, 0.f);
    if (use_tc && !st.has_dw && res < 0 && st.act == kActNone && is_view(cur)) {
      int sib = -1;
      for (size_t j = 0; j < m.ops.size() && sib < 0; ++j) {
        const TfOp& o2 = m.ops[j];
        if ((int)j == ci || done[j] || o2.code != kOpConv2D || o2.in[0] != conv.in[0]) continue;
        const TfTensor& w2t = m.tensors[o2.in[1]];
        if (w2t.shape.size() != 4 || w2t.shape[1] != 1 || w2t.shape[2] != 1 || w2t.shape[3] != Cin) continue;
        if (o2.stride_h != 1 || o2.stride_w != 1 || o2.act != 0 || !is_view(o2.out[0])) continue;
        sib = (int)j;
      }
      if (sib >= 0) {
        const TfOp& o2 = m.ops[sib];
        const int sib_out = o2.out[0];
        std::vector<float> w2, b2;
        bool ok2 = m.const_f32(o2.in[1], &w2);
        if (ok2 && o2.in.size() > 2 && o2.in[2] >= 0) ok2 = m.const_f32(o2.in[2], &b2);
        const int C2n = m.tensors[o2.in[1]].shape[0];
        b2.resize(C2n, 0.f);
        const bool this_primary = st.Cout % 4 == 0 && (C2n % 4 != 0 || st.Cout >= C2n);
        const int Cp = this_primary ? st.Cout : C2n, Cq = this_primary ? C2n : st.Cout;
        const int p_out = this_primary ? cur : sib_out, q_out = this_primary ? sib_out : cur;
        const bool vec_ok = views[p_out].off % 4 == 0 && P.out_elems[views[p_out].root] % 4 == 0;
        if (ok2 && Cp % 4 == 0 && vec_ok) {
          std::vector<float> wm, bm;
          const std::vector<float>& wp = this_primary ? w : w2;
          const std::vector<float>& wq = this_primary ? w2 : w;
          const std::vector<float>& bp = this_primary ? b : b2;
          const std::vector<float>& bq = this_primary ? b2 : b;
          wm.insert(wm.end(), wp.begin(), wp.end()); wm.insert(wm.end(), wq.begin(), wq.end());
          bm.insert(bm.end(), bp.begin(), bp.end()); bm.insert(bm.end(), bq.begin(), bq.end());
          PStep t = st;
          t.Cout = Cp + Cq; t.c1 = Cp; t.c2 = Cq;
          if (plan_tc(&t, Cin, OH, OW, tf32_exact(wm) ? 1 : 2) && plan_ws(&t, OH, OW)) {
            st.Cout = Cp + Cq; st.c1 = Cp; st.c2 = Cq;
            plan_columns(&st);
            const std::string nm = m.tensors[p_out].name + "+" + m.tensors[q_out].name;
            F->st = st;
            F->st.name = nm;
            F->out_tf = p_out; F->out2_tf = q_out;
            done[sib] = 1;
            fused_outputs.push_back(sib_out);
            w.swap(wm); b.swap(bm);
          }
        }
      }
    }
    const int w_parts = tf32_exact(w) ? 1 : 2;
    bool tc = false;
    if (use_tc) {
      PStep t = F->st;
      res_c_hint = res >= 0 ? m.tensors[res].dim(3) : 0;
      tc = plan_tc(&t, Cin, OH, OW, w_parts) && plan_ws(&t, OH, OW);
      res_c_hint = 0;
      if (tc) F->st = t;
    }
    if (F->st.c2 > 0 && F->st.kind != kStepBlockWs) return fail("internal: merged heads need the warp-specialised kernel");
    const PStep& fs = F->st;
    if (tc) {
      const size_t SBO = (size_t)(fs.K8 / 4) * 128, LBO = 128;
      std::vector<float> wb((size_t)w_parts * fs.Npad * fs.K8, 0.f);
      for (int n = 0; n < fs.Cout; ++n)
        for (int k = 0; k < Cin; ++k) {
          size_t o = ((size_t)(n >> 3) * SBO + (size_t)(k >> 2) * LBO + (size_t)(n & 7) * 16 + (size_t)(k & 3) * 4) / 4;
          split_w(w[(size_t)n * Cin + k], w_parts, &wb[o], &wb[o + (w_parts > 1 ? (size_t)fs.Npad * fs.K8 : 0)]);
        }
      F->st.w = push(wb, wb.size());
      F->st.bias = push(b, (size_t)fs.Npad + 8);
      if (alpha_tf >= 0 && !pack_alpha(alpha_tf, (size_t)fs.Npad + 8, &F->st.alpha)) return false;
    } else {
      std::vector<float> wk((size_t)st.KP * st.CoutP, 0.f);
      for (int co = 0; co < st.Cout; ++co)
        for (int c = 0; c < Cin; ++c) wk[(size_t)c * st.CoutP + co] = w[(size_t)co * Cin + c];
      size_t padded = (size_t)st.nchunks * st.NC + 8;
      F->st.w = push(wk, wk.size());
      F->st.bias = push(b, padded);
      if (alpha_tf >= 0 && !pack_alpha(alpha_tf, padded, &F->st.alpha)) return false;
    }
    if (st.has_dw) {
      const TfOp& dw = m.ops[absorbed[0]];
      std::vector<float> dwv, dbv;
      if (!m.const_f32(dw.in[1], &dwv) || !m.const_f32(dw.in[2], &dbv)) return fail("depthwise weights are not constant");
      const int kp = tc ? fs.K8 : st.KP;
      std::vector<float> dk((size_t)9 * kp, 0.f);
      for (int t = 0; t < 9; ++t)
        for (int c = 0; c < Cin; ++c) dk[(size_t)t * kp + c] = dwv[(size_t)t * Cin + c];
      F->st.dww = push(dk, dk.size());
      F->st.dwb = push(dbv, kp);
    }
    F->st.macs = (double)OH * OW * ((double)Cin * st.Cout + (st.has_dw ? 9.0 * Cin : 0.0));
    if (tc && F->st.kind == kStepBlockWs) plan_ts(&F->st, st_in, OH, OW, alpha_tf >= 0);
    return true;
  }

  void plan_ts(PStep* st, const TfTensor& in, int OH, int OW, bool prelu) {
    static const int want = [] { const char* e = std::getenv("FDT_TS"); return e ? std::atoi(e) : 1; }();
    if (!want || !st->has_dw || st->c2 > 0 || st->w_parts != 1 || prelu) return;
    if (st->act != kActRelu && st->act != kActNone) return;
    const int Cin = in.dim(3), K16 = ru(Cin, 16), Npad = ru(st->Cout, 16);
    if (K16 > 64 || Npad > 64) return;
    if (st->dws == 1 ? (OH % 16 || OW % 16 || st->dpt != 1 || st->dpl != 1)
                     : (OH % 8 || OW % 16 || st->dpt != 0 || st->dpl != 0 || in.dim(1) != 2 * OH || in.dim(2) != 2 * OW)) return;
    int res = 0;
    if (st->res_mode != 0) {
      if (st->res_mode != 1) return;
      res = st->res_pool ? 2 : 1;
      if ((res == 2) != (st->dws == 2)) return;
    }
    const size_t SBO8 = (size_t)(st->K8 / 4) * 128, SBO16 = (size_t)(K16 / 8) * 128;
    std::vector<uint16_t> wh((size_t)Npad * K16, 0);
    for (int n = 0; n < st->Cout; ++n)
      for (int k = 0; k < Cin; ++k) {
        const float v = P.blob[(size_t)st->w + ((size_t)(n >> 3) * SBO8 + (size_t)(k >> 2) * 128 + (size_t)(n & 7) * 16 + (size_t)(k & 3) * 4) / 4];
        const uint16_t hbits = f32_to_f16(v);
        if (f16_to_f32(hbits) != v) return;
        wh[((size_t)(n >> 3) * SBO16 + (size_t)(k >> 3) * 128 + (size_t)(n & 7) * 16 + (size_t)(k & 7) * 2) / 2] = hbits;
      }
    std::vector<float> rec(wh.size() / 2 + (size_t)10 * K16, 0.f);
    std::memcpy(rec.data(), wh.data(), wh.size() * 2);
    float* dw = rec.data() + wh.size() / 2;
    for (int k = 0; k < 9; ++k)
      for (int c = 0; c < Cin; ++c) dw[(size_t)k * K16 + c] = P.blob[(size_t)st->dww + (size_t)k * st->K8 + c];
    for (int c = 0; c < Cin; ++c) dw[(size_t)9 * K16 + c] = P.blob[(size_t)st->dwb + c];
    std::vector<float> bias((size_t)Npad, 0.f);
    for (int n = 0; n < st->Cout; ++n) bias[n] = P.blob[(size_t)st->bias + n];
    const int KS = odd_quads(ru(Cin, 4));
    const int stage_bytes = st->dws == 1 ? (18 * 18 * KS * 4 + 127) / 128 * 128 : 2 * ((17 * 17 * KS * 4 + 127) / 128 * 128);
    const size_t head = rec.size() * 4 + (size_t)Npad * 4 + 32 * 8 + 256;
    int ns = (int)(((size_t)220 * 1024 - head) / stage_bytes);
    if (ns < 2) return;
    if (ns > 4) ns = 4;
    st->ts_rec = push(rec, rec.size());
    st->ts_bias = push(bias, bias.size());
    st->ts_rec_bytes = (int)(rec.size() * 4);
    st->ts_k16 = K16; st->ts_npad = Npad; st->ts_ks = KS; st->ts_ns = ns; st->ts_stage_bytes = stage_bytes;
    st->ts_res = res; st->ts_relu = st->act == kActRelu ? 1 : 0;
    st->TH = st->dws == 1 ? 16 : 8; st->TW = 16; st->G = 1;
    st->smem = head + (size_t)ns * stage_bytes;
    st->kind = kStepBlockTs;
  }

  static void split_w(float v, int parts, float* hi, float* lo) {
    if (parts == 1) { *hi = v; return; }
    uint32_t u;
    std::memcpy(&u, &v, 4);
    u &= 0xFFFFE000u;
    float h;
    std::memcpy(&h, &u, 4);
    *hi = h;
    *lo = v - h;
  }

  static bool tf32_exact(const std::vector<float>& w) {
    for (float v : w) {
      uint32_t u;
      std::memcpy(&u, &v, 4);
      if (u & 0x1FFFu) return false;
    }
    return true;
  }

  bool plan_tc(PStep* st, int Cin, int OH, int OW, int w_parts) {
    PStep s = *st;
    s.w_parts = w_parts;
    s.K8 = ru(Cin, 8);
    s.Npad = ru(s.Cout, 16);
    if (s.Npad > 128 || s.K8 > 256) return false;
    s.KS = s.K8 + (((s.K8 / 4) % 2 == 0) ? 4 : 0);
    s.tmem_cols = 32;
    while (s.tmem_cols < s.Npad) s.tmem_cols *= 2;
    for (int Pn = 128; Pn >= 32; Pn /= 2) {
      const size_t cap = (size_t)220 * 1024;
      s.TM = 1; s.NPG = Pn;
      int bestTH = 0, bestTW = 0, bestG = 1;
      double best = -1;
      if (OH * OW <= Pn && OW <= 30) {
        bestTH = OH; bestTW = OW; bestG = std::min(63, Pn / (OH * OW));
      } else {
        for (int TW = std::min(std::min(OW, Pn), 30); TW >= 1; --TW) {
          int TH = std::min(std::min(OH, Pn / TW), 30);
          if (TH < 1) continue;
          double tiles = (double)((OH + TH - 1) / TH) * ((OW + TW - 1) / TW);
          double util = (double)OH * OW / (tiles * Pn);
          double halo = (double)((TH - 1) * s.dws + 3) * ((TW - 1) * s.dws + 3) / ((double)TH * TW * s.dws * s.dws);
          double score = util / (s.has_dw ? halo : 1.0);
          if (score > best + 1e-9) { best = score; bestTH = TH; bestTW = TW; }
        }
      }
      s.TH = bestTH; s.TW = bestTW; s.G = bestG;
      s.IH = s.has_dw ? (s.TH - 1) * s.dws + 3 : s.TH;
      s.IW = s.has_dw ? (s.TW - 1) * s.dws + 3 : s.TW;
      s.tilesY = (OH + s.TH - 1) / s.TH;
      s.tilesX = (OW + s.TW - 1) / s.TW;
      int nslots = s.G * s.TH * s.TW;
      s.a_rows = ru(nslots, 8);
      s.RS = 1;
      for (int rs : {8, 4, 2}) if (s.TH % rs == 0 && s.G * (s.K8 / 4) * (s.TH / rs) * s.TW >= 256) { s.RS = rs; break; }
      if (s.IH > 63 || s.IW > 63 || s.G > 63 || nslots > 255) continue;
      size_t head = (size_t)s.w_parts * s.Npad * s.K8 + 2 * (size_t)s.Npad + (s.has_dw ? 10 * (size_t)s.K8 : 0);
      size_t a = 2 * (size_t)s.a_rows * s.K8;
      size_t in = (size_t)s.G * s.IH * s.IW * s.KS;
      size_t need_tail = (size_t)(128 - s.a_rows) * s.K8;
      if (in < need_tail) in = need_tail;
      in = (in + 3) / 4 * 4;
      size_t n_chunks = (size_t)s.G * s.IH * s.IW * (s.K8 / 4);
      size_t n_items = s.has_dw ? (size_t)s.G * (s.K8 / 4) * (s.TH / s.RS) * s.TW : 0;
      size_t smem1 = (head + a + in) * 4 + (n_chunks + n_items) * 8 + 128;
      size_t smem2 = smem1 + in * 4;
      bool dbl = smem2 <= 113 * 1024 || (smem1 > 113 * 1024 && smem2 <= 220 * 1024);
      s.nbuf = dbl ? 2 : 1;
      s.smem = dbl ? smem2 : smem1;
      if (s.smem <= cap) { *st = s; return true; }
    }
    return false;
  }

  int res_c_hint = 0;
  bool plan_ws(PStep* st, int OH, int OW) {
    constexpr int max_ns = 6, max_na = 4;
    PStep s = *st;
    {
      int ks = s.K8;
      if (s.res_mode == 1 && cs(s.Cout) > ks) ks = cs(s.Cout);
      if ((ks / 4) % 2 == 0) ks += 4;
      s.KS = ks;
    }
    s.nt = 4 * s.Npad <= 512 ? 4 : 2;
    s.tmem_cols = 32;
    while (s.tmem_cols < s.nt * s.Npad) s.tmem_cols *= 2;
    if (s.tmem_cols > 512) return false;
    const size_t cap = (size_t)225 * 1024;
    for (int Pn = 128; Pn >= 32; Pn /= 2) {
      s.TM = 1; s.NPG = Pn;
      int bestTH = 0, bestTW = 0, bestG = 1;
      double best = -1;
      if (OH * OW <= Pn) {
        bestTH = OH; bestTW = OW; bestG = Pn / (OH * OW);
      } else {
        for (int TW = std::min(OW, Pn); TW >= 1; --TW) {
          int TH = std::min(OH, Pn / TW);
          if (TH < 1) continue;
          double tiles = (double)((OH + TH - 1) / TH) * ((OW + TW - 1) / TW);
          double util = (double)OH * OW / (tiles * Pn);
          double halo = (double)((TH - 1) * s.dws + 3) * ((TW - 1) * s.dws + 3) / ((double)TH * TW * s.dws * s.dws);
          double score = util / (s.has_dw ? halo : 1.0);
          if (score > best + 1e-9) { best = score; bestTH = TH; bestTW = TW; }
        }
      }
      s.TH = bestTH; s.TW = bestTW; s.G = bestG;
      s.IH = s.has_dw ? (s.TH - 1) * s.dws + 3 : s.TH;
      s.IW = s.has_dw ? (s.TW - 1) * s.dws + 3 : s.TW;
      s.tilesY = (OH + s.TH - 1) / s.TH;
      s.tilesX = (OW + s.TW - 1) / s.TW;
      if (s.IH > 256 || s.IW > 256 || s.G > 256 || s.KS > 256) continue;
      s.a_rows = std::min(128, ru(s.G * s.TH * s.TW, 8));
      s.RS = 1; s.nd = 8;
      if (s.has_dw) {
        double best_cost = 1e30;
        for (int nd : {12, 8}) {
          for (int rs : {1, 2, 4}) {
            if (s.TH % rs || rs > (nd == 12 ? 2 : 4)) continue;
            int items = s.G * (s.K8 / 4) * (s.TH / rs) * s.TW;
            int m = (items + nd * 32 - 1) / (nd * 32);
            int rows = s.dws == 1 ? rs + 2 : 2 * rs + 1;
            double cost = m * ((m > 1 ? 14 : 0) + 3.0 * rows + 50.0 * rs + 10);
            if (cost < best_cost - 1e-9) { best_cost = cost; s.RS = rs; s.nd = nd; }
          }
        }
      }
      if (s.has_dw && s.dws == 1 && s.res_mode == 2 && !s.res_pool && ru(s.Cout, 4) <= 32 && s.K8 <= 16) {
        s.nd = 8;
        int items = s.G * (s.K8 / 4) * s.TH * s.TW;
        s.RS = (items > 256 && s.TH % 2 == 0) ? 2 : 1;
        if (s.G * (s.K8 / 4) * (s.TH / s.RS) * s.TW > 256 && s.TH % 4 == 0) s.RS = 4;
      }
      size_t n_items = s.has_dw ? (size_t)s.G * (s.K8 / 4) * (s.TH / s.RS) * s.TW : 0;
      size_t head = ((size_t)s.w_parts * s.Npad * s.K8 + 2 * (size_t)s.Npad + (s.has_dw ? 10 * (size_t)s.K8 : 0)) * 4 + (n_items + 1) / 2 * 8 + 48 * 8 + 128;
      size_t a_bytes = (size_t)2 * s.a_rows * s.K8 * 4;
      size_t in_bytes = ((size_t)s.G * s.IH * s.IW * s.KS * 4 + 127) / 128 * 128;
      s.deint = (s.has_dw && s.dws == 2 && s.dpt == 0 && s.dpl == 0 && (s.IW & 1)) ? 1 : 0;
      s.PW = (s.IW + 1) / 2;
      if (s.deint) {
        const size_t plane = ((size_t)s.G * s.IH * s.PW * s.KS * 4 + 127) / 128 * 128;
        s.plane_floats = (int)(plane / 4);
        in_bytes = 2 * plane;
      }
      static const int want_no = [] { const char* e = std::getenv("FDT_WS_NO"); return e ? std::atoi(e) : 0; }();
      const int couts = cs(s.Cout);
      s.KSo = ((couts / 4) % 2 == 0) ? couts + 4 : couts;
      const size_t out_bytes = ((size_t)s.G * s.TH * s.TW * s.KSo * 4 + 127) / 128 * 128;
      const bool can_tma_out = s.KSo <= 256;
      static const int combos[10][2] = {{4, 6}, {4, 5}, {4, 4}, {2, 5}, {2, 4}, {2, 3}, {2, 2}, {1, 2}, {1, 1}, {0, 0}};
      static const int prefs[5][2] = {{2, 2}, {1, 2}, {2, 1}, {1, 1}, {0, 1}};
      size_t res_bytes = 0;
      int want_nr = 0;
      s.nr = 0; s.KSr = 0; s.res_stage_floats = 0;
      if (s.res_mode == 2 && s.c2 == 0) {
        const int m = s.res_pool ? 2 : 1;
        s.KSr = odd_quads(ru(s.Cout, 4));
        if (s.res_pool && res_c_hint > 0) s.KSr = odd_quads(ru(res_c_hint, 4));
        if (s.KSr <= 256 && m * s.TW <= 256 && m * s.TH <= 256) {
          res_bytes = ((size_t)s.G * (m * s.TH) * (m * s.TW) * s.KSr * 4 + 127) / 128 * 128;
          want_nr = 3;
        }
      }
      for (const auto& pr : prefs) {
        const int no = pr[0];
        if (no > want_no || (no > 0 && (!can_tma_out || s.c2 > 0))) continue;
        for (const auto& c : combos) {
          if (c[0] == 0 || c[0] > max_na || c[1] > max_ns || c[1] < pr[1]) continue;
          size_t total = head + c[0] * a_bytes + c[1] * in_bytes + no * out_bytes;
          int nr = 0;
          if (want_nr && no == 0) {
            nr = (int)std::min<size_t>(4, total < cap ? (cap - total) / res_bytes : 0);
            if (nr < 2) { if (c[0] > 1 || c[1] > 2) continue; nr = 0; }
            total += (size_t)nr * res_bytes;
          }
          const size_t over = (size_t)(128 - s.a_rows) * s.K8 * 4, after = c[1] * in_bytes + no * out_bytes;
          if (over > after) total += over - after;
          if (total > cap) continue;
          s.na = c[0]; s.ns = c[1]; s.no = no;
          s.nr = nr; s.res_stage_floats = (int)(res_bytes / 4);
          s.in_stage_floats = (int)(in_bytes / 4);
          s.out_stage_floats = (int)(out_bytes / 4);
          s.smem = total;
          s.kind = kStepBlockWs;
          *st = s;
          return true;
        }
      }
    }
    return false;
  }

  std::vector<int> fused_outputs;
  bool is_output_of_fused(int tf) const {
    return std::find(fused_outputs.begin(), fused_outputs.end(), tf) != fused_outputs.end();
  }

  bool plan_spatial(PStep* s, int OH, int OW) {
    for (int attempt = 0; attempt < 2; ++attempt) {
      int Pn = s->TM * s->NPG;
      int bestTH = 0, bestTW = 0, bestG = 1;
      double best = -1;
      if (OH * OW <= Pn) {
        bestTH = OH; bestTW = OW; bestG = Pn / (OH * OW);
      } else {
        for (int TW = std::min(OW, Pn); TW >= 1; --TW) {
          int TH = std::min(OH, Pn / TW);
          if (TH < 1) continue;
          double tiles = (double)((OH + TH - 1) / TH) * ((OW + TW - 1) / TW);
          double util = (double)OH * OW / (tiles * Pn);
          double halo = (double)((TH - 1) * s->dws + 3) * ((TW - 1) * s->dws + 3) / ((double)TH * TW * s->dws * s->dws);
          double score = util / (s->has_dw ? halo : 1.0);
          if (score > best + 1e-9) { best = score; bestTH = TH; bestTW = TW; }
        }
      }
      s->TH = bestTH; s->TW = bestTW; s->G = bestG;
      s->IH = s->has_dw ? (s->TH - 1) * s->dws + 3 : s->TH;
      s->IW = s->has_dw ? (s->TW - 1) * s->dws + 3 : s->TW;
      s->tilesY = (OH + s->TH - 1) / s->TH;
      s->tilesX = (OW + s->TW - 1) / s->TW;
      size_t in_elems = (size_t)s->G * s->IH * s->IW * s->KS;
      size_t a_elems = (size_t)Pn * s->KS;
      size_t floats = s->has_dw ? in_elems + a_elems : std::max(in_elems, a_elems);
      floats += (size_t)s->KP * s->NC;
      s->smem = floats * 4;
      if (s->smem <= kSmemLimit) return true;
      if (s->NPG % 2 == 0 && attempt == 0) s->NPG /= 2; else break;
    }
    return false;
  }

  bool analyse_dense(int ci, Fused* F) {
    const TfOp& conv = m.ops[ci];
    const TfTensor& wt = m.tensors[conv.in[1]];
    const TfTensor& it = m.tensors[conv.in[0]];
    const TfTensor& ot = m.tensors[conv.out[0]];
    if (wt.shape.size() != 4 || it.shape.size() != 4 || conv.dil_h != 1 || conv.dil_w != 1) return false;
    if (conv.act != 0 && conv.act != 1) return false;
    PStep st;
    st.kind = kStepGemmConv;
    st.kh = wt.shape[1]; st.kw = wt.shape[2];
    st.sh = conv.stride_h; st.sw = conv.stride_w;
    int Cin = wt.shape[3];
    st.Cout = wt.shape[0];
    if (use_tc && conv.padding == 1 && st.kh == it.dim(1) && st.kw == it.dim(2) && ot.numel() == st.Cout && conv.act == 0 &&
        !is_view(conv.in[0]) && Cin % 4 == 0 && Cin == it.dim(3) && (st.kh * st.kw * Cin) % 16 == 0 && st.kh * st.kw * Cin <= 384) {
      std::vector<float> w, b;
      if (!m.const_f32(conv.in[1], &w)) return fail("conv weights are not constant");
      if (conv.in.size() > 2 && conv.in[2] >= 0) { if (!m.const_f32(conv.in[2], &b)) return fail("conv bias is not constant"); }
      b.resize(st.Cout, 0.f);
      st.kind = kStepFcTc;
      st.K = st.kh * st.kw * Cin;
      st.K8 = st.K;
      st.w_parts = f16_exact(w) ? 1 : 2;
      float scale = 1.f, wsc = 1.f;
      if (st.w_parts == 2) {
        float mx = 0.f;
        for (float v : w) mx = std::max(mx, std::fabs(v));
        if (mx > 0.f) { int e; std::frexp(mx, &e); scale = std::ldexp(1.f, 14 - e); }
      }
      const int ntile = (st.Cout + 127) / 128;
      std::vector<float> rec;
      for (int tI = 0; tI < ntile; ++tI) {
        std::vector<float> r1 = pack_w_f16(w, std::min(128, st.Cout - tI * 128), st.K, 128, st.K, st.w_parts, &wsc, scale, tI * 128);
        rec.insert(rec.end(), r1.begin(), r1.end());
      }
      st.ts_rec_bytes = st.w_parts * 128 * st.K * 2;
      st.out_scale = 1.0 / (double)scale;
      st.w = push(rec, rec.size());
      st.bias = push(b, b.size() + 8);
      st.smem = (size_t)st.ts_rec_bytes + 256;
      st.act = kActNone;
      done[ci] = 1;
      st.macs = (double)st.K * st.Cout;
      st.name = m.tensors[conv.out[0]].name;
      F->ok = true;
      F->st = st;
      F->src_tf = conv.in[0];
      F->out_tf = conv.out[0];
      fused_outputs.push_back(conv.out[0]);
      return true;
    }
    if (conv.padding == 0) { same_pad(it.dim(1), st.kh, st.sh, &st.pt); same_pad(it.dim(2), st.kw, st.sw, &st.pl); }
    st.K = st.kh * st.kw * Cin;
    st.KP = ru(st.K, 4);
    st.KS = smem_stride(st.KP);
    plan_columns(&st);
    {
      bool fit = false;
      PStep best = st;
      int best_chunks = 1 << 30;
      for (int P = 128; P >= 32; P /= 2) {
        PStep c = st;
        plan_columns(&c);
        for (;;) {
          c.TM = (c.NC / 4) <= 12 && P >= 128 ? 4 : (P >= 128 ? 8 : 4);
          c.NPG = P / c.TM;
          c.smem = ((size_t)P * c.KS + (size_t)c.KP * c.NC) * 4;
// ... 888 lines not shown
```

face_detection_tflite_b200/csrc/plan.h:

```cpp
#pragma once
#include <map>
#include <string>
#include <vector>

#include "tail_layer.h"
#include "tflite_model.h"

namespace fdt {

struct PTensor {
  int tf = -1;
  int H = 1, W = 1, C = 1, Cs = 1;
  long long istride = 0;
  int root = -1;
  long long view_off = 0;
  long long arena_off = -1;
  int def_step = -1, last_use = -1;
  bool materialized = false;
  bool is_input = false;
};

enum StepKind { kStepNormalize, kStepNaiveConv, kStepGemmConv, kStepDwPw, kStepAdd, kStepAct, kStepPadC,
                kStepMaxPool, kStepResize, kStepStem, kStepBlockWs, kStepStemWs, kStepTailWs, kStepFcTc, kStepBlockTs };

struct PStep {
  StepKind kind = kStepAct;
  std::string name;
  int in = -1, in2 = -1, out = -1;
  int kh = 1, kw = 1, sh = 1, sw = 1, pt = 0, pl = 0, act = 0, depthwise = 0;
  bool in_u8 = false;
  bool has_dw = false;
  int dws = 1, dpt = 0, dpl = 0, res_pool = 0, res_mode = 0;
  long long w = -1, bias = -1, alpha = -1, dww = -1, dwb = -1;
  int K = 0, KP = 0, KS = 0, Cout = 0, CoutP = 0, NC = 0, nchunks = 0, NPG = 0, TM = 0;
  int TH = 0, TW = 0, G = 1, IH = 0, IW = 0, tilesX = 1, tilesY = 1;
  size_t smem = 0;
  int K8 = 0, Npad = 0, a_rows = 0, RS = 1, tmem_cols = 0, w_parts = 1, nbuf = 1;
  double out_scale = 1.0;
  int ns = 0, na = 0, nd = 8, nt = 2, in_stage_floats = 0;
  int no = 0, KSo = 0, out_stage_floats = 0;
  int nr = 0, KSr = 0, res_stage_floats = 0;
  int deint = 0, plane_floats = 0, PW = 0;
  int out2 = -1, c1 = 0, c2 = 0;
  int fh = 1, fw = 1, align = 0, half = 0;
  std::vector<int> extra_out;
  long long ts_rec = -1, ts_bias = -1;
  int ts_rec_bytes = 0, ts_k16 = 0, ts_npad = 0, ts_ks = 0, ts_ns = 0, ts_stage_bytes = 0, ts_res = 0, ts_relu = 0;
  std::vector<TailLayerD> tail;
  std::vector<int> tail_outs;
  int tail_nbuf = 0, tail_buf_off[kTailMaxBufs] = {0}, tail_buf_ks[kTailMaxBufs] = {0}, tail_buf_px[kTailMaxBufs] = {0};
  std::vector<TailBlk> tail_blks;
  std::vector<int> tail_rsrc;
  int tail_wide = 0, tail_bias_floats = 0;
  int tail_act_floats = 0, tail_in_bytes = 0, tail_last_a = 0, tail_wbuf = 0, tail_wdepth = 2, tail_tbuf = 0;
  double macs = 0;
};

struct Plan {
  std::vector<PTensor> tensors;
  std::vector<PStep> steps;
  std::vector<float> blob;
  std::map<int, int> tf2pt;
  int input = -1, in_h = 0, in_w = 0;
  std::vector<int> outputs;
  std::vector<long long> out_elems;
  long long arena_per_image = 0;
  int fuse_level = 1;

  bool build(const TfModel& m, int fuse_level, std::string* err, bool use_tc = true);
  std::string describe() const;
};

}
```

Before: 776,600.

## Enlarge stride-1 block tiles to four M-tiles for row halo reuse

Adds a four-M-tile (32-row) variant of the stride-1 fused depthwise+pointwise tensor-core block kernel for small-channel layers. It loads a taller input box per tile so the depthwise stage reuses each loaded row across up to four output rows, and it packs TMEM columns more densely to fit. It also replaces the half-split residual computation with an f16 FMA and folds the bias into the first depthwise FMA using paired f32x2 FMAs. The cost is larger stages, so fewer pipeline stages fit, and there are fewer tiles for grid parallelism.

```diff
diff --git a/face_detection_tflite_b200/csrc/engine.cu b/face_detection_tflite_b200/csrc/engine.cu
--- a/face_detection_tflite_b200/csrc/engine.cu
+++ b/face_detection_tflite_b200/csrc/engine.cu
@@ -274,7 +274,7 @@
         p.out = out.p; p.out_istride = out.istride; p.OH = out.H; p.OW = out.W; p.CoutS = out.Cs;
         p.rec = blob + st.ts_rec; p.bias = blob + st.ts_bias; p.rec_bytes = st.ts_rec_bytes;
         p.Cin = iv.C; p.K16 = st.ts_k16; p.Npad = st.ts_npad; p.KS = st.ts_ks;
-        p.stride = st.dws; p.res = st.ts_res; p.relu = st.ts_relu;
+        p.stride = st.dws; p.rows = st.ts_rows; p.res = st.ts_res; p.relu = st.ts_relu;
         p.wide = (out.Cs % 8 == 0 && out.istride % 8 == 0 && ((size_t)out.p % 32 == 0)) ? 1 : 0;
         p.ns = st.ts_ns; p.stage_bytes = st.ts_stage_bytes; p.smem_bytes = st.smem;
         {
diff --git a/face_detection_tflite_b200/csrc/kernels.h b/face_detection_tflite_b200/csrc/kernels.h
--- a/face_detection_tflite_b200/csrc/kernels.h
+++ b/face_detection_tflite_b200/csrc/kernels.h
@@ -199,6 +199,7 @@
   int rec_bytes;
   int Cin, K16, Npad, KS;
   int stride;
+  int rows;
   int res;
   int relu, wide;
   int ns, stage_bytes;
diff --git a/face_detection_tflite_b200/csrc/kernels_tail.cu b/face_detection_tflite_b200/csrc/kernels_tail.cu
--- a/face_detection_tflite_b200/csrc/kernels_tail.cu
+++ b/face_detection_tflite_b200/csrc/kernels_tail.cu
@@ -66,11 +66,16 @@
   asm("cvt.rn.satfinite.f16x2.f32 %0, %1, %2;" : "=r"(d) : "f"(e1), "f"(e0));
   return d;
 }
+template <int H>
+__device__ __forceinline__ float sub_half(float e, uint32_t h2) {
+  float d;
+  if (H) asm("{\n\t.reg .b16 l, h, m;\n\tmov.b32 {l, h}, %1;\n\tmov.b16 m, 0xBC00;\n\tfma.rn.f32.f16 %0, h, m, %2;\n\t}" : "=f"(d) : "r"(h2), "f"(e));
+  else asm("{\n\t.reg .b16 l, h, m;\n\tmov.b32 {l, h}, %1;\n\tmov.b16 m, 0xBC00;\n\tfma.rn.f32.f16 %0, l, m, %2;\n\t}" : "=f"(d) : "r"(h2), "f"(e));
+  return d;
+}
 __device__ __forceinline__ void split_store_tmem(uint32_t taddr_hi, const float4& a) {
   const uint32_t h0 = pack_h2(a.x, a.y), h1 = pack_h2(a.z, a.w);
-  const __half2 hh0 = *reinterpret_cast<const __half2*>(&h0), hh1 = *reinterpret_cast<const __half2*>(&h1);
-  const float2 f0 = __half22float2(hh0), f1 = __half22float2(hh1);
-  const uint32_t l0 = pack_h2(a.x - f0.x, a.y - f0.y), l1 = pack_h2(a.z - f1.x, a.w - f1.y);
+  const uint32_t l0 = pack_h2(sub_half<0>(a.x, h0), sub_half<1>(a.y, h0)), l1 = pack_h2(sub_half<0>(a.z, h1), sub_half<1>(a.w, h1));
   asm volatile("tcgen05.st.sync.aligned.32x32b.x2.b32 [%0], {%1, %2};" ::"r"(taddr_hi), "r"(h0), "r"(h1) : "memory");
   asm volatile("tcgen05.st.sync.aligned.32x32b.x2.b32 [%0], {%1, %2};" ::"r"(taddr_hi + 64u), "r"(l0), "r"(l1) : "memory");
 }
diff --git a/face_detection_tflite_b200/csrc/kernels_ts.cu b/face_detection_tflite_b200/csrc/kernels_ts.cu
--- a/face_detection_tflite_b200/csrc/kernels_ts.cu
+++ b/face_detection_tflite_b200/csrc/kernels_ts.cu
@@ -50,6 +50,15 @@
       : "+f"(a.x), "+f"(a.y), "+f"(a.z), "+f"(a.w)
       : "f"(v.x), "f"(v.y), "f"(v.z), "f"(v.w), "f"(w.x), "f"(w.y), "f"(w.z), "f"(w.w));
 }
+__device__ __forceinline__ void fma4_to(float4& d, const float4& v, const float4& w, const float4& c) {
+  asm("{\n\t.reg .b64 ra, rv, rw;\n\t"
+      "mov.b64 ra, {%12, %13};\n\tmov.b64 rv, {%4, %5};\n\tmov.b64 rw, {%8, %9};\n\t"
+      "fma.rn.f32x2 ra, rv, rw, ra;\n\tmov.b64 {%0, %1}, ra;\n\t"
+      "mov.b64 ra, {%14, %15};\n\tmov.b64 rv, {%6, %7};\n\tmov.b64 rw, {%10, %11};\n\t"
+      "fma.rn.f32x2 ra, rv, rw, ra;\n\tmov.b64 {%2, %3}, ra;\n\t}"
+      : "=f"(d.x), "=f"(d.y), "=f"(d.z), "=f"(d.w)
+      : "f"(v.x), "f"(v.y), "f"(v.z), "f"(v.w), "f"(w.x), "f"(w.y), "f"(w.z), "f"(w.w), "f"(c.x), "f"(c.y), "f"(c.z), "f"(c.w));
+}
 __device__ __forceinline__ float4 max4(const float4& a, const float4& b) {
   return make_float4(fmaxf(a.x, b.x), fmaxf(a.y, b.y), fmaxf(a.z, b.z), fmaxf(a.w, b.w));
 }
@@ -58,10 +67,16 @@
   asm("cvt.rn.satfinite.f16x2.f32 %0, %1, %2;" : "=r"(d) : "f"(e1), "f"(e0));
   return d;
 }
+template <int H>
+__device__ __forceinline__ float sub_half(float e, uint32_t h2) {
+  float d;
+  if (H) asm("{\n\t.reg .b16 l, h, m;\n\tmov.b32 {l, h}, %1;\n\tmov.b16 m, 0xBC00;\n\tfma.rn.f32.f16 %0, h, m, %2;\n\t}" : "=f"(d) : "r"(h2), "f"(e));
+  else asm("{\n\t.reg .b16 l, h, m;\n\tmov.b32 {l, h}, %1;\n\tmov.b16 m, 0xBC00;\n\tfma.rn.f32.f16 %0, l, m, %2;\n\t}" : "=f"(d) : "r"(h2), "f"(e));
+  return d;
+}
 __device__ __forceinline__ void split_store_tmem(uint32_t taddr_hi, uint32_t lo_off, const float4& a) {
   const uint32_t h0 = pack_h2(a.x, a.y), h1 = pack_h2(a.z, a.w);
-  const float2 f0 = __half22float2(*reinterpret_cast<const __half2*>(&h0)), f1 = __half22float2(*reinterpret_cast<const __half2*>(&h1));
-  const uint32_t l0 = pack_h2(a.x - f0.x, a.y - f0.y), l1 = pack_h2(a.z - f1.x, a.w - f1.y);
+  const uint32_t l0 = pack_h2(sub_half<0>(a.x, h0), sub_half<1>(a.y, h0)), l1 = pack_h2(sub_half<0>(a.z, h1), sub_half<1>(a.w, h1));
   asm volatile("tcgen05.st.sync.aligned.32x32b.x2.b32 [%0], {%1, %2};" ::"r"(taddr_hi), "r"(h0), "r"(h1) : "memory");
   asm volatile("tcgen05.st.sync.aligned.32x32b.x2.b32 [%0], {%1, %2};" ::"r"(taddr_hi + lo_off), "r"(l0), "r"(l1) : "memory");
 }
@@ -74,15 +89,18 @@
   asm volatile("st.global.v8.f32 [%0], {%1, %2, %3, %4, %5, %6, %7, %8};" ::"l"(p), "f"(a.x), "f"(a.y), "f"(a.z), "f"(a.w), "f"(b.x), "f"(b.y), "f"(b.z), "f"(b.w) : "memory");
 }
 
-__device__ __forceinline__ uint32_t col_d(int slot, int t) { return (uint32_t)(slot * 2 + t) * 64u; }
-__device__ __forceinline__ uint32_t col_a(int slot, int t) { return 256u + (uint32_t)(slot * 2 + t) * 64u; }
-
-template <int S, int KSC>
+template <int NT> __device__ __forceinline__ uint32_t col_d(int slot, int t) {
+  return NT == 4 ? (uint32_t)(slot * 4 + t) * 32u : (uint32_t)(slot * 2 + t) * 64u;
+}
+template <int NT> __device__ __forceinline__ uint32_t col_a(int slot, int t) { return 256u + col_d<NT>(slot, t); }
+template <int NT> __host__ __device__ constexpr uint32_t lo_cols() { return NT == 4 ? 16u : 32u; }
+
+template <int S, int KSC, int NT>
 __global__ void __launch_bounds__(kThreads, 1) k_block_ts(const __grid_constant__ CUtensorMap tmap, const __grid_constant__ BlockTsP p, int B) {
   extern __shared__ __align__(128) unsigned char smem_raw[];
   __shared__ uint32_t tmem_base_s;
-  constexpr int NT = S == 1 ? 2 : 1;
-  constexpr int TH = S == 1 ? 16 : 8, TW = 16;
+  static_assert(S == 1 ? (NT == 2 || NT == 4) : NT == 1, "M-tiles per output tile");
+  constexpr int TH = 8 * NT, TW = 16;
   constexpr int IW = S == 1 ? 18 : 17;
   const int tid = threadIdx.x, warp = tid >> 5, lane = tid & 31;
   float* sRec = reinterpret_cast<float*>(smem_raw);
@@ -125,7 +143,7 @@
     const int L = lq * 32 + lane;
     const int yy = L >> 4, x = L & 15;
     const uint32_t tm_lane = tmem_base + ((uint32_t)(lq * 32) << 16);
-    const uint32_t win = (uint32_t)((2 * yy) * IW + x) * ks_b;
+    const uint32_t win = (uint32_t)((S == 1 ? NT * yy : 2 * yy) * IW + x) * ks_b;
     const int nq = p.K16 >> 2, nq_real = (p.Cin + 3) >> 2, ks_q = KS >> 2;
     const uint32_t bias_a = smem_u32(sBias), zero_a = bar0 + 192u;
     const int couts = p.CoutS, nc8 = (couts + 7) >> 3;
@@ -137,65 +155,65 @@
       mbar_wait(d_full + 8u * (uint32_t)slot, (uint32_t)((i >> 1) & 1));
       asm volatile("tcgen05.fence::after_thread_sync;" ::: "memory");
       const uint32_t st_a = ring_a + (uint32_t)stage * stage_b + win;
-      float* const orow0 = p.out + (size_t)b * p.out_istride + (uint32_t)(((ty * TH + (S == 1 ? 2 * yy : yy)) * p.OW + tx * TW + x) * couts);
+      float* const orow0 = p.out + (size_t)b * p.out_istride + (uint32_t)(((ty * TH + (S == 1 ? NT * yy : yy)) * p.OW + tx * TW + x) * couts);
       const uint32_t orow_step = (uint32_t)(p.OW * couts);
+      auto unit = [&](auto ngc, auto lgc, int c8, uint32_t dcol, float* orow, uint32_t res_a) {
+        constexpr int NG = decltype(ngc)::value;
+        constexpr int lg = decltype(lgc)::value;
+        uint32_t u[8 * NG];
+        if (NG == 2)
+          asm volatile(
+              "tcgen05.ld.sync.aligned.32x32b.x16.b32 {%0, %1, %2, %3, %4, %5, %6, %7, %8, %9, %10, %11, %12, %13, %14, %15}, [%16];"
+              : "=r"(u[0]), "=r"(u[1]), "=r"(u[2]), "=r"(u[3]), "=r"(u[4]), "=r"(u[5]), "=r"(u[6]), "=r"(u[7]),
+                "=r"(u[8 * (NG - 1)]), "=r"(u[8 * (NG - 1) + 1]), "=r"(u[8 * (NG - 1) + 2]), "=r"(u[8 * (NG - 1) + 3]),
+                "=r"(u[8 * (NG - 1) + 4]), "=r"(u[8 * (NG - 1) + 5]), "=r"(u[8 * (NG - 1) + 6]), "=r"(u[8 * (NG - 1) + 7])
+              : "r"(dcol + 8u * (uint32_t)c8));
+        else
+          asm volatile("tcgen05.ld.sync.aligned.32x32b.x8.b32 {%0, %1, %2, %3, %4, %5, %6, %7}, [%8];"
+                       : "=r"(u[0]), "=r"(u[1]), "=r"(u[2]), "=r"(u[3]), "=r"(u[4]), "=r"(u[5]), "=r"(u[6]), "=r"(u[7])
+                       : "r"(dcol + 8u * (uint32_t)c8));
+        float4 bv[2 * NG], rv[2 * NG];
+#pragma unroll
+        for (int j = 0; j < 2 * NG; ++j) {
+          const int cq = 2 * c8 + j;
+          const uint32_t qo = 16u * (uint32_t)cq;
+          bv[j] = lds4(bias_a + qo);
+          rv[j] = make_float4(0.f, 0.f, 0.f, 0.f);
+          if (S == 2) {
+            rv[j] = rvp[lg + (j >> 1)][j & 1];
+          } else if (S == 1) {
+            rv[j] = lds4(p.res == 1 && cq < ks_q ? res_a + qo : zero_a);
+          } else if (p.res == 2) {
+            if (cq < ks_q) rv[j] = max4(max4(lds4(res_a + qo), lds4(res_a + plane_b + qo)), max4(lds4(res_a + row_b + qo), lds4(res_a + row_b + plane_b + qo)));
+          }
+        }
+        asm volatile("tcgen05.wait::ld.sync.aligned;" ::: "memory");
+        float4 v[2 * NG];
+#pragma unroll
+        for (int j = 0; j < 2 * NG; ++j) {
+          v[j] = make_float4(__uint_as_float(u[4 * j]) + bv[j].x + rv[j].x, __uint_as_float(u[4 * j + 1]) + bv[j].y + rv[j].y,
+                             __uint_as_float(u[4 * j + 2]) + bv[j].z + rv[j].z, __uint_as_float(u[4 * j + 3]) + bv[j].w + rv[j].w);
+          if (p.relu) v[j] = max4(v[j], make_float4(0.f, 0.f, 0.f, 0.f));
+        }
+#pragma unroll
+        for (int k = 0; k < NG; ++k) {
+          const int c = 8 * (c8 + k);
+          if (c + 8 <= couts) {
+            if (p.wide) stg8(orow + c, v[2 * k], v[2 * k + 1]);
+            else { *reinterpret_cast<float4*>(orow + c) = v[2 * k]; *reinterpret_cast<float4*>(orow + c + 4) = v[2 * k + 1]; }
+          } else if (c + 4 <= couts) {
+            *reinterpret_cast<float4*>(orow + c) = v[2 * k];
+          }
+        }
+      };
 #pragma unroll
       for (int t = 0; t < NT; ++t) {
-        float* orow = orow0 + (t ? orow_step : 0u);
+        float* orow = orow0 + (uint32_t)t * orow_step;
         const uint32_t res_a = S == 1 ? st_a + (uint32_t)(t + 1) * row_b + ks_b : st_a;
-        const uint32_t dcol = tm_lane + col_d(slot, t);
-        auto unit = [&](auto ngc, auto lgc, int c8) {
-          constexpr int NG = decltype(ngc)::value;
-          constexpr int lg = decltype(lgc)::value;
-          uint32_t u[8 * NG];
-          if (NG == 2)
-            asm volatile(
-                "tcgen05.ld.sync.aligned.32x32b.x16.b32 {%0, %1, %2, %3, %4, %5, %6, %7, %8, %9, %10, %11, %12, %13, %14, %15}, [%16];"
-                : "=r"(u[0]), "=r"(u[1]), "=r"(u[2]), "=r"(u[3]), "=r"(u[4]), "=r"(u[5]), "=r"(u[6]), "=r"(u[7]),
-                  "=r"(u[8 * (NG - 1)]), "=r"(u[8 * (NG - 1) + 1]), "=r"(u[8 * (NG - 1) + 2]), "=r"(u[8 * (NG - 1) + 3]),
-                  "=r"(u[8 * (NG - 1) + 4]), "=r"(u[8 * (NG - 1) + 5]), "=r"(u[8 * (NG - 1) + 6]), "=r"(u[8 * (NG - 1) + 7])
-                : "r"(dcol + 8u * (uint32_t)c8));
-          else
-            asm volatile("tcgen05.ld.sync.aligned.32x32b.x8.b32 {%0, %1, %2, %3, %4, %5, %6, %7}, [%8];"
-                         : "=r"(u[0]), "=r"(u[1]), "=r"(u[2]), "=r"(u[3]), "=r"(u[4]), "=r"(u[5]), "=r"(u[6]), "=r"(u[7])
-                         : "r"(dcol + 8u * (uint32_t)c8));
-          float4 bv[2 * NG], rv[2 * NG];
-#pragma unroll
-          for (int j = 0; j < 2 * NG; ++j) {
-            const int cq = 2 * c8 + j;
-            const uint32_t qo = 16u * (uint32_t)cq;
-            bv[j] = lds4(bias_a + qo);
-            rv[j] = make_float4(0.f, 0.f, 0.f, 0.f);
-            if (S == 2) {
-              rv[j] = rvp[lg + (j >> 1)][j & 1];
-            } else if (S == 1) {
-              rv[j] = lds4(p.res == 1 && cq < ks_q ? res_a + qo : zero_a);
-            } else if (p.res == 2) {
-              if (cq < ks_q) rv[j] = max4(max4(lds4(res_a + qo), lds4(res_a + plane_b + qo)), max4(lds4(res_a + row_b + qo), lds4(res_a + row_b + plane_b + qo)));
-            }
-          }
-          asm volatile("tcgen05.wait::ld.sync.aligned;" ::: "memory");
-          float4 v[2 * NG];
-#pragma unroll
-          for (int j = 0; j < 2 * NG; ++j) {
-            v[j] = make_float4(__uint_as_float(u[4 * j]) + bv[j].x + rv[j].x, __uint_as_float(u[4 * j + 1]) + bv[j].y + rv[j].y,
-                               __uint_as_float(u[4 * j + 2]) + bv[j].z + rv[j].z, __uint_as_float(u[4 * j + 3]) + bv[j].w + rv[j].w);
-            if (p.relu) v[j] = max4(v[j], make_float4(0.f, 0.f, 0.f, 0.f));
-          }
-#pragma unroll
-          for (int k = 0; k < NG; ++k) {
-            const int c = 8 * (c8 + k);
-            if (c + 8 <= couts) {
-              if (p.wide) stg8(orow + c, v[2 * k], v[2 * k + 1]);
-              else { *reinterpret_cast<float4*>(orow + c) = v[2 * k]; *reinterpret_cast<float4*>(orow + c + 4) = v[2 * k + 1]; }
-            } else if (c + 4 <= couts) {
-              *reinterpret_cast<float4*>(orow + c) = v[2 * k];
-            }
-          }
-        };
-        if (gn >= 2) unit(std::integral_constant<int, 2>(), std::integral_constant<int, 0>(), g0);
-        if (gn == 1) unit(std::integral_constant<int, 1>(), std::integral_constant<int, 0>(), g0);
-        if (gn == 3) unit(std::integral_constant<int, 1>(), std::integral_constant<int, 2>(), g0 + 2);
+        const uint32_t dcol = tm_lane + col_d<NT>(slot, t);
+        if (gn >= 2) unit(std::integral_constant<int, 2>(), std::integral_constant<int, 0>(), g0, dcol, orow, res_a);
+        if (gn == 1) unit(std::integral_constant<int, 1>(), std::integral_constant<int, 0>(), g0, dcol, orow, res_a);
+        if (gn == 3) unit(std::integral_constant<int, 1>(), std::integral_constant<int, 2>(), g0 + 2, dcol, orow, res_a);
       }
       asm volatile("tcgen05.fence::before_thread_sync;" ::: "memory");
       __syncwarp();
@@ -210,9 +228,39 @@
       const int slot = i & 1;
       mbar_wait(in_full + 8u * (uint32_t)stage, in_phase);
       const uint32_t st_a = ring_a + (uint32_t)stage * stage_b + win;
-      const uint32_t acol0 = tm_lane + col_a(slot, 0), acol1 = tm_lane + col_a(slot, 1);
+      const uint32_t acol0 = tm_lane + col_a<NT>(slot, 0), acol1 = tm_lane + col_a<NT>(slot, 1);
       for (int q = g; q < nq; q += 3) {
         if (q >= nq_real && i >= 2) break;
+        if constexpr (NT == 4) {
+          float4 a[4];
+          if (q < nq_real) {
+            const float4* cw = reinterpret_cast<const float4*>(p.dw) + 10 * q;
+            float4 w[9];
+#pragma unroll
+            for (int k = 0; k < 9; ++k) w[k] = cw[k];
+            const float4 bias = cw[9];
+            const uint32_t pa = st_a + 16u * (uint32_t)q;
+#pragma unroll
+            for (int r = 0; r < 6; ++r) {
+              float4 v[3];
+#pragma unroll
+              for (int c = 0; c < 3; ++c) v[c] = lds4(pa + (uint32_t)r * row_b + (uint32_t)c * ks_b);
+#pragma unroll
+              for (int t = r < 2 ? 0 : r - 2; t <= (r < 3 ? r : 3); ++t)
+#pragma unroll
+                for (int c = 0; c < 3; ++c) {
+                  if (t == r && c == 0) fma4_to(a[t], v[c], w[0], bias);
+                  else fma4(a[t], v[c], w[3 * (r - t) + c]);
+                }
+            }
+          } else {
+#pragma unroll
+            for (int t = 0; t < 4; ++t) a[t] = make_float4(0.f, 0.f, 0.f, 0.f);
+          }
+#pragma unroll
+          for (int t = 0; t < 4; ++t) split_store_tmem(tm_lane + col_a<NT>(slot, t) + 2u * (uint32_t)q, lo_cols<NT>(), a[t]);
+          continue;
+        }
         float4 a0 = make_float4(0.f, 0.f, 0.f, 0.f), a1 = a0;
         if (q < nq_real) {
           const uint32_t qo = 16u * (uint32_t)q;
@@ -248,8 +296,8 @@
             for (int k = 0; k < 9; ++k) fma4(a0, lds4(pa + (uint32_t)(k / 3) * row_b + col2_b[k % 3]), w[k]);
           }
         }
-        split_store_tmem(acol0 + 2u * (uint32_t)q, 32u, a0);
-        if (S == 1) split_store_tmem(acol1 + 2u * (uint32_t)q, 32u, a1);
+        split_store_tmem(acol0 + 2u * (uint32_t)q, lo_cols<NT>(), a0);
+        if (S == 1) split_store_tmem(acol1 + 2u * (uint32_t)q, lo_cols<NT>(), a1);
       }
       asm volatile("tcgen05.wait::st.sync.aligned;" ::: "memory");
       asm volatile("tcgen05.fence::before_thread_sync;" ::: "memory");
@@ -285,7 +333,7 @@
         const int b = at.b, ty = at.ty, tx = at.tx;
         if (i >= NS) mbar_wait_idle(in_empty + 8u * (uint32_t)stage, empty_phase);
         const uint32_t bar = in_full + 8u * (uint32_t)stage;
-        mbar_expect_tx(bar, (uint32_t)((S == 1 ? 18 * 18 : 2 * 17 * 17) * KS) * 4u);
+        mbar_expect_tx(bar, (uint32_t)((S == 1 ? 18 * (TH + 2) : 2 * 17 * 17) * KS) * 4u);
         const int ix0 = S == 1 ? tx * TW - 1 : tx * TW * 2, iy0 = S == 1 ? ty * TH - 1 : ty * TH * 2;
         asm volatile("cp.async.bulk.tensor.4d.shared::cluster.global.mbarrier::complete_tx::bytes [%0], [%1, {%2, %3, %4, %5}], [%6];"
                      ::"r"(ring_a + (uint32_t)stage * stage_b), "l"(&tmap), "r"(0), "r"(ix0), "r"(iy0), "r"(b), "r"(bar) : "memory");
@@ -310,13 +358,13 @@
         asm volatile("tcgen05.fence::after_thread_sync;" ::: "memory");
 #pragma unroll
         for (int t = 0; t < NT; ++t) {
-          const uint32_t dcol = tmem_base + col_d(slot, t), acol = tmem_base + col_a(slot, t);
+          const uint32_t dcol = tmem_base + col_d<NT>(slot, t), acol = tmem_base + col_a<NT>(slot, t);
           uint32_t acc = 0u;
 #pragma unroll 1
           for (int part = 0; part < 2; ++part)
 #pragma unroll 1
             for (int ks = 0; ks < ksteps; ++ks) {
-              mma_ts_f16(dcol, acol + 32u * (uint32_t)part + 8u * (uint32_t)ks, b_lo0 + 16u * (uint32_t)ks, b_hi, idesc, acc);
+              mma_ts_f16(dcol, acol + lo_cols<NT>() * (uint32_t)part + 8u * (uint32_t)ks, b_lo0 + 16u * (uint32_t)ks, b_hi, idesc, acc);
               acc = 1u;
             }
         }
@@ -348,10 +396,10 @@
 }
 
 bool ts_tensor_map(const BlockTsP& p, int cap, CUtensorMap* out) {
-  typedef std::tuple<const void*, int, int, int, int, int, int, long long> Key;
+  typedef std::tuple<const void*, int, int, int, int, int, int, int, long long> Key;
   static std::mutex mu;
   static std::map<Key, CUtensorMap> cache;
-  Key key(p.in, cap, p.H, p.W, p.CinS, p.KS, p.stride, p.in_istride);
+  Key key(p.in, cap, p.H, p.W, p.CinS, p.KS, p.stride, p.rows, p.in_istride);
   std::lock_guard<std::mutex> g(mu);
   auto it = cache.find(key);
   if (it != cache.end()) { *out = it->second; return true; }
@@ -359,7 +407,7 @@
   if (!enc) return false;
   cuuint64_t gdim[4] = {(cuuint64_t)p.CinS, (cuuint64_t)p.W, (cuuint64_t)p.H, (cuuint64_t)cap};
   cuuint64_t gstr[3] = {(cuuint64_t)p.CinS * 4, (cuuint64_t)p.W * p.CinS * 4, (cuuint64_t)p.in_istride * 4};
-  cuuint32_t box[4] = {(cuuint32_t)p.KS, p.stride == 1 ? 18u : 33u, p.stride == 1 ? 18u : 17u, 1u};
+  cuuint32_t box[4] = {(cuuint32_t)p.KS, p.stride == 1 ? 18u : 33u, p.stride == 1 ? 8u * (cuuint32_t)p.rows + 2u : 17u, 1u};
   cuuint32_t estr[4] = {1, p.stride == 1 ? 1u : 2u, 1, 1};
   CUtensorMap tm;
   CUresult r = enc(&tm, CU_TENSOR_MAP_DATA_TYPE_FLOAT32, 4, const_cast<float*>(p.in), gdim, gstr, box, estr,
@@ -372,7 +420,7 @@
   return true;
 }
 
-template <int S, int KSC>
+template <int S, int KSC, int NT>
 bool launch_ts(const CUtensorMap& tm, const BlockTsP& p, int B, cudaStream_t s) {
   static std::mutex mu;
   static std::map<int, size_t> cur;
@@ -383,13 +431,13 @@
     std::lock_guard<std::mutex> g(mu);
     size_t& c = cur[dev];
     if (p.smem_bytes > c) {
-      if (cudaFuncSetAttribute(k_block_ts<S, KSC>, cudaFuncAttributeMaxDynamicSharedMemorySize, (int)p.smem_bytes) != cudaSuccess) return false;
+      if (cudaFuncSetAttribute(k_block_ts<S, KSC, NT>, cudaFuncAttributeMaxDynamicSharedMemorySize, (int)p.smem_bytes) != cudaSuccess) return false;
       c = p.smem_bytes;
     }
   }
-  const int ntiles = B * (p.OW / 16) * (p.OH / (S == 1 ? 16 : 8));
+  const int ntiles = B * (p.OW / 16) * (p.OH / (8 * NT));
   const int grid = std::max(1, std::min(ntiles, sms));
-  k_block_ts<S, KSC><<<grid, kThreads, p.smem_bytes, s>>>(tm, p, B);
+  k_block_ts<S, KSC, NT><<<grid, kThreads, p.smem_bytes, s>>>(tm, p, B);
   return true;
 }
 
@@ -403,22 +451,23 @@
   if (B <= 0) return true;
   CUtensorMap tm;
   if (!ts_tensor_map(p, cap, &tm)) return false;
+  if (p.stride == 1 && p.rows == 4) return p.KS == 28 ? launch_ts<1, 28, 4>(tm, p, B, s) : launch_ts<1, 0, 4>(tm, p, B, s);
   if (p.stride == 1) {
     switch (p.KS) {
-      case 28: return launch_ts<1, 28>(tm, p, B, s);
-      case 36: return launch_ts<1, 36>(tm, p, B, s);
-      case 44: return launch_ts<1, 44>(tm, p, B, s);
-      case 52: return launch_ts<1, 52>(tm, p, B, s);
-      default: return launch_ts<1, 0>(tm, p, B, s);
+      case 28: return launch_ts<1, 28, 2>(tm, p, B, s);
+      case 36: return launch_ts<1, 36, 2>(tm, p, B, s);
+      case 44: return launch_ts<1, 44, 2>(tm, p, B, s);
+      case 52: return launch_ts<1, 52, 2>(tm, p, B, s);
+      default: return launch_ts<1, 0, 2>(tm, p, B, s);
     }
   }
   switch (p.KS) {
-    case 28: return launch_ts<2, 28>(tm, p, B, s);
-    case 36: return launch_ts<2, 36>(tm, p, B, s);
-    case 44: return launch_ts<2, 44>(tm, p, B, s);
-    case 52: return launch_ts<2, 52>(tm, p, B, s);
-    default: return launch_ts<2, 0>(tm, p, B, s);
-  }
-}
-
-}
+    case 28: return launch_ts<2, 28, 1>(tm, p, B, s);
+    case 36: return launch_ts<2, 36, 1>(tm, p, B, s);
+    case 44: return launch_ts<2, 44, 1>(tm, p, B, s);
+    case 52: return launch_ts<2, 52, 1>(tm, p, B, s);
+    default: return launch_ts<2, 0, 1>(tm, p, B, s);
+  }
+}
+
+}
diff --git a/face_detection_tflite_b200/csrc/plan.cpp b/face_detection_tflite_b200/csrc/plan.cpp
--- a/face_detection_tflite_b200/csrc/plan.cpp
+++ b/face_detection_tflite_b200/csrc/plan.cpp
@@ -448,8 +448,16 @@
     std::vector<float> bias((size_t)Npad, 0.f);
     for (int n = 0; n < st->Cout; ++n) bias[n] = P.blob[(size_t)st->bias + n];
     const int KS = odd_quads(ru(Cin, 4));
-    const int stage_bytes = st->dws == 1 ? (18 * 18 * KS * 4 + 127) / 128 * 128 : 2 * ((17 * 17 * KS * 4 + 127) / 128 * 128);
     const size_t head = rec.size() * 4 + (size_t)Npad * 4 + 32 * 8 + 256;
+    static const int rows_max = [] { const char* e = std::getenv("FDT_TS_ROWS"); return e && std::atoi(e) == 2 ? 2 : 4; }();
+    const int stage4 = (18 * 34 * KS * 4 + 127) / 128 * 128;
+    const int rows = st->dws == 1 && rows_max == 4 && K16 <= 32 && Npad <= 32 &&
+#ifdef FDT_EXP_COUT8
+                     st->Cout % 8 == 0 &&
+#endif
+                     OH % 32 == 0 &&
+                     ((size_t)220 * 1024 - head) / stage4 >= 3 ? 4 : 2;
+    const int stage_bytes = st->dws == 1 ? (18 * (8 * rows + 2) * KS * 4 + 127) / 128 * 128 : 2 * ((17 * 17 * KS * 4 + 127) / 128 * 128);
     int ns = (int)(((size_t)220 * 1024 - head) / stage_bytes);
     if (ns < 2) return;
     if (ns > 4) ns = 4;
@@ -457,8 +465,8 @@
     st->ts_bias = push(bias, bias.size());
     st->ts_rec_bytes = (int)(rec.size() * 4);
     st->ts_k16 = K16; st->ts_npad = Npad; st->ts_ks = KS; st->ts_ns = ns; st->ts_stage_bytes = stage_bytes;
-    st->ts_res = res; st->ts_relu = st->act == kActRelu ? 1 : 0;
-    st->TH = st->dws == 1 ? 16 : 8; st->TW = 16; st->G = 1;
+    st->ts_res = res; st->ts_relu = st->act == kActRelu ? 1 : 0; st->ts_rows = rows;
+    st->TH = st->dws == 1 ? 8 * rows : 8; st->TW = 16; st->G = 1;
     st->smem = head + (size_t)ns * stage_bytes;
     st->kind = kStepBlockTs;
   }
diff --git a/face_detection_tflite_b200/csrc/plan.h b/face_detection_tflite_b200/csrc/plan.h
--- a/face_detection_tflite_b200/csrc/plan.h
+++ b/face_detection_tflite_b200/csrc/plan.h
@@ -45,7 +45,7 @@
   int fh = 1, fw = 1, align = 0, half = 0;
   std::vector<int> extra_out;
   long long ts_rec = -1, ts_bias = -1;
-  int ts_rec_bytes = 0, ts_k16 = 0, ts_npad = 0, ts_ks = 0, ts_ns = 0, ts_stage_bytes = 0, ts_res = 0, ts_relu = 0;
+  int ts_rec_bytes = 0, ts_k16 = 0, ts_npad = 0, ts_ks = 0, ts_ns = 0, ts_stage_bytes = 0, ts_res = 0, ts_relu = 0, ts_rows = 2;
   std::vector<TailLayerD> tail;
   std::vector<int> tail_outs;
   int tail_nbuf = 0, tail_buf_off[kTailMaxBufs] = {0}, tail_buf_ks[kTailMaxBufs] = {0}, tail_buf_px[kTailMaxBufs] = {0};
```

Result: faster. 794,400, median of 6 (+2.3%).
